# Lab-LVM/imagenet-models

Hardware: AMD Instinct MI355X
Metric: images/sec (whole node) GA-ConvNeXt-T 3x224x224 bf16 training step (higher is better)
Workload: dtype bf16; 1 GPU; ga_convnext_tiny_768 train step (fwd + GA loss lam=-0.8 + bwd + all-reduce + adamw lr=0), batch 256/GPU, drop_path 0.2, synthetic 3x224x224; global_batch=256, parallelism=dp1, dist_backend=none, grad_exchange=torch, allreduce_buckets=0

## Files before the change

imagenet-models_amd/_lib.py:

```python
import ctypes as C
import os

_HERE = os.path.dirname(os.path.abspath(__file__))
LIB_PATH = os.environ.get('GAEXT_LIB') or os.path.join(_HERE, 'csrc', 'libgaext.so')

GA_F32, GA_BF16 = 0, 1
ACT_NONE, ACT_GELU, ACT_RELU = 0, 1, 2
A_PLAIN, A_PATCH2, A_STEM4_NCHW, A_CONV3, A_CONV3S2, A_NEIGH2 = 0, 1, 2, 3, 4, 5
C_PLAIN, C_UNPATCH2 = 0, 1

vp, i32, i64, f32 = C.c_void_p, C.c_int, C.c_int64, C.c_float


class GemmDesc(C.Structure):
    _fields_ = [
        ('M', i32), ('N', i32), ('K', i32), ('batch', i32), ('dtype', i32),
        ('A', vp), ('lda', i64), ('strideA', i64), ('a_batch_mod', i32), ('a_kind', i32),
        ('a_H', i32), ('a_W', i32), ('a_C', i32), ('a_act', i32),
        ('B', vp), ('ldb', i64), ('strideB', i64),
        ('C', vp), ('ldc', i64), ('strideC', i64), ('c_kind', i32),
        ('c_H', i32), ('c_W', i32), ('c_C', i32), ('c_f32', i32), ('C2', vp), ('c2_mode', i32),
        ('alpha', f32), ('bias', vp), ('strideBias', i64), ('act', i32),
        ('H', vp), ('ldh', i64), ('strideH', i64), ('h_is_deriv', i32),
        ('rowscale', vp), ('rows_per_scale', i32),
        ('R', vp), ('ldr', i64), ('strideR', i64), ('relu_after', i32),
        ('colsum', vp), ('colsumsq', vp), ('strideCol', i64),
    ]


class WgradDesc(C.Structure):
    _fields_ = [
        ('M', i32), ('N', i32), ('K', i32), ('batch', i32), ('dtype', i32),
        ('Y', vp), ('ldy', i64), ('strideY', i64),
        ('X', vp), ('ldx', i64), ('strideX', i64), ('x_batch_mod', i32), ('x_kind', i32),
        ('x_H', i32), ('x_W', i32), ('x_C', i32), ('x_act', i32),
        ('dW', vp), ('ldw', i64), ('strideW', i64),
        ('dbias', vp), ('strideDbias', i64),
        ('alpha', f32), ('split_m', i32), ('accumulate', i32), ('workspace', vp), ('ws_bytes', i64),
    ]


class WprepDesc(C.Structure):
    _fields_ = [
        ('w', vp), ('G', i32), ('Co', i32), ('Ci', i32), ('KH', i32), ('KW', i32),
        ('rs', vp), ('cs', vp), ('row_perm', vp), ('dtype', i32),
        ('out', vp), ('ldo', i64), ('outT', vp), ('ldt', i64), ('flip', i32), ('stem', i32), ('t_cols', i32),
    ]


class WunfoldDesc(C.Structure):
    _fields_ = [
        ('G', vp), ('ldg', i64), ('gb', vp), ('W', vp), ('b', vp), ('rs', vp), ('cs', vp), ('v', vp), ('row_perm', vp),
        ('N', i32), ('Ci', i32), ('KH', i32), ('KW', i32), ('stem', i32),
        ('dW', vp), ('db', vp), ('d_rs', vp), ('d_cs', vp), ('d_v', vp),
    ]


class SmallDesc(C.Structure):
    _fields_ = [('kind', i32), ('y', vp), ('x', vp), ('a', f32), ('n', i64), ('R', i32), ('C', i32), ('accumulate', i32),
                ('b', vp), ('rs', vp), ('v', vp), ('row_perm', vp)]


class CswinAttnDesc(C.Structure):
    _fields_ = [('B', i32), ('reso', i32), ('C', i32), ('heads', i32), ('nbranch', i32),
                ('Hs', i32 * 2), ('Ws', i32 * 2), ('lepe_w', vp * 2), ('lepe_b', vp * 2),
                ('scale', f32), ('dtype', i32), ('qkv', vp), ('ldq', i64), ('out', vp), ('ldo', i64)]


class MlpDesc(C.Structure):
    _fields_ = [('X', vp), ('ldx', i64), ('W1', vp), ('ldw1', i64), ('b1', vp), ('W2', vp), ('ldw2', i64), ('b2', vp),
                ('R', vp), ('ldr', i64), ('rowscale', vp), ('rows_per_scale', i32), ('Y', vp), ('ldy', i64),
                ('M', i64), ('C', i32), ('H', i32), ('dtype', i32)]


class MlpBwdDesc(C.Structure):
    _fields_ = [('X', vp), ('ldx', i64), ('DY', vp), ('lddy', i64), ('W1', vp), ('ldw1', i64), ('b1', vp),
                ('W2T', vp), ('ldw2t', i64), ('W1T', vp), ('ldw1t', i64), ('A', vp), ('lda', i64), ('DH', vp), ('lddh', i64),
                ('DX', vp), ('lddx', i64), ('M', i64), ('C', i32), ('H', i32), ('dtype', i32),
                ('dW1', vp), ('ldw', i64), ('db1', vp), ('partials', vp), ('partials_bytes', C.c_size_t), ('max_blocks', i32)]


class SmallLinearDesc(C.Structure):
    _fields_ = [('rows', i32), ('groups', i32), ('Ng', i32), ('Kg', i32), ('A', vp), ('lda', i64), ('a_gstride', i64), ('a_perm', vp),
                ('W', vp), ('bias', vp), ('col_scale', vp), ('rowscale', vp), ('rows_per_scale', i32), ('R', vp), ('ldr', i64),
                ('Y', vp), ('ldy', i64), ('Yraw', vp), ('dtype', i32)]


class AttnDesc(C.Structure):
    _fields_ = [('B', i32), ('N', i32), ('H', i32), ('hd', i32), ('scale', f32), ('dtype', i32), ('qkv', vp), ('ldq', i64),
                ('out', vp), ('ldo', i64), ('lse', vp)]


_SIGS = {
    'ga_version': ([], i32),
    'ga_last_error': ([C.c_char_p, C.c_size_t], i32),
    'ga_device_info': ([C.POINTER(i32), C.POINTER(i32), C.POINTER(i32)], i32),
    'ga_comm_unique_id': ([vp], i32),
    'ga_comm_init': ([C.POINTER(vp), i32, i32, vp], i32),
    'ga_comm_destroy': ([vp], i32),
    'ga_comm_info': ([vp, C.POINTER(i32), C.POINTER(i32)], i32),
    'ga_allreduce_workspace': ([i64, i32], C.c_size_t),
    'ga_allreduce_bucket': ([vp, vp, i64, i32, f32, vp, C.c_size_t, vp], i32),
    'ga_reduce_scatter_bucket': ([vp, vp, vp, i64, f32, vp], i32),
    'ga_allgather_bucket': ([vp, vp, vp, i64, vp], i32),
    'ga_comm_broadcast': ([vp, vp, i64, i32, vp], i32),
    'ga_set_knob': ([C.c_char_p, i32], i32),
    'ga_unset_knob': ([C.c_char_p], i32),
    'ga_config_string': ([C.c_char_p, C.c_size_t], i32),
    'ga_gemm': ([C.POINTER(GemmDesc), vp], i32),
    'ga_wgrad': ([C.POINTER(WgradDesc), vp], i32),
    'ga_weight_prep': ([C.POINTER(WprepDesc), vp], i32),
    'ga_bias_fold': ([vp, vp, vp, vp, vp, vp, i32, i32, vp], i32),
    'ga_weight_unfold': ([C.POINTER(WunfoldDesc), vp], i32),
    'ga_dwconv7_fwd': ([vp, vp, vp, vp, i32, i32, i32, i32, i32, vp], i32),
    'ga_dwconv7_bwd_data': ([vp, vp, vp, vp, i32, i32, i32, i32, i32, vp], i32),
    'ga_dwconv7_bwd_data2': ([vp, vp, vp, vp, vp, vp, i32, i32, i32, i32, i32, vp], i32),
    'ga_dwconv7_bwd_weight': ([vp, vp, vp, vp, i32, i32, i32, i32, i32, vp, C.c_size_t, vp], i32),
    'ga_dwconv7_bwd_weight_workspace': ([i32, i32, i32, i32, i32], C.c_size_t),
    'ga_dwconv3_fwd': ([vp, vp, vp, i32, i32, i32, i32, i32, vp, vp, i32, vp], i32),
    'ga_dwconv3_bwd_data': ([vp, vp, vp, i32, i32, i32, i32, i32, i32, vp], i32),
    'ga_dwconv3_bwd_weight': ([vp, vp, vp, i32, i32, i32, i32, i32, i32, vp, C.c_size_t, vp], i32),
    'ga_dwconv3_bwd_weight_workspace': ([i32, i32, i32, i32, i32, i32], C.c_size_t),
    'ga_maxpool3s2_fwd': ([vp, vp, vp, i32, i32, i32, i32, i32, vp], i32),
    'ga_maxpool3s2_bwd': ([vp, vp, vp, i32, i32, i32, i32, i32, i32, vp], i32),
    'ga_bn_gelu_fwd': ([vp, vp, vp, vp, i64, i32, i32, vp], i32),
    'ga_bn_gelu_bwd_workspace': ([i64, i32], C.c_size_t),
    'ga_bn_gelu_bwd_reduce': ([vp, vp, vp, vp, vp, vp, vp, vp, i64, i32, i32, vp, C.c_size_t, vp], i32),
    'ga_bn_gelu_bwd_apply': ([vp, vp, vp, vp, vp, vp, vp, vp, vp, i64, vp, i64, i32, i32, vp], i32),
    'ga_se_bn_fwd': ([vp, i32, vp, vp, vp, vp, vp, vp, vp, vp, vp, vp, vp, vp, vp, vp, i32, i32, i32, i32, vp], i32),
    'ga_se_bn_bwd': ([vp, vp, vp, vp, vp, vp, vp, vp, i32, vp, vp, vp, vp, vp, vp, vp, vp, vp, vp, vp, vp, vp, vp, vp, vp, vp, vp, vp,
                      vp, vp, i32, i32, i32, vp], i32),
    'ga_se_residual_fwd': ([vp, vp, vp, vp, vp, vp, vp, vp, vp, i32, i32, i32, i32, vp], i32),
    'ga_se_residual_bwd_a': ([vp, vp, vp, vp, vp, vp, vp, vp, i32, i32, i32, i32, vp], i32),
    'ga_se_residual_bwd_b': ([vp, vp, vp, vp, vp, vp, vp, vp, vp, vp, vp, i32, i32, i32, i32, vp], i32),
    'ga_subsample2_fwd': ([vp, vp, i32, i32, i32, i32, i32, vp], i32),
    'ga_subsample2_bwd': ([vp, vp, i32, i32, i32, i32, i32, i32, vp], i32),
    'ga_wgrad_workspace': ([C.POINTER(WgradDesc)], C.c_size_t),
    'ga_layernorm_fwd': ([vp, vp, vp, vp, vp, vp, i64, i32, f32, i32, vp], i32),
    'ga_layernorm_bwd': ([vp, vp, vp, vp, vp, vp, vp, vp, vp, i64, i32, i32, i32, vp], i32),
    'ga_layernorm_bwd_dp': ([vp, vp, vp, vp, vp, vp, vp, vp, vp, i64, i32, i32, vp, vp, i64, i32, vp], i32),
    'ga_bn_finalize': ([vp, vp, i64, vp, vp, f32, f32, vp, vp, vp, vp, vp, vp, i32, i32, vp], i32),
    'ga_affine_act': ([vp, vp, vp, vp, vp, i64, vp, i64, i32, i32, i32, i64, vp], i32),
    'ga_bn_bwd_reduce': ([vp, vp, vp, vp, vp, vp, i64, vp, vp, i64, i32, i32, i64, vp], i32),
    'ga_bn_bwd_apply': ([vp, vp, vp, vp, vp, vp, vp, vp, vp, i64, i64, vp, i64, i32, i32, i64, i64, vp], i32),
    'ga_pool_concat_fwd': ([vp, vp, i32, i32, i32, i32, i32, i32, i32, i32, i32, i32, vp], i32),
    'ga_pool_concat_bwd': ([vp, vp, vp, i32, i32, i32, i32, i32, i32, i32, i32, i32, i32, vp], i32),
    'ga_spatial_sum': ([vp, vp, vp, i32, i32, i32, f32, i32, vp], i32),
    'ga_se_mlp_fwd': ([vp, vp, vp, vp, vp, vp, vp, i32, i32, i32, vp], i32),
    'ga_se_mlp_bwd': ([vp, vp, vp, vp, vp, vp, vp, f32, vp, vp, vp, vp, i32, i32, i32, vp], i32),
    'ga_chan_scale': ([vp, vp, vp, vp, i32, i32, i32, i32, vp], i32),
    'ga_gram_pack_fwd': ([vp, vp, vp, i32, i32, i32, i32, i32, vp], i32),
    'ga_gram_pack_bwd': ([vp, vp, vp, vp, i32, i32, i32, i32, i32, vp], i32),
    'ga_gram_f64_fwd_workspace': ([i32, i32], C.c_size_t),
    'ga_gram_f64_bwd_workspace': ([i32, i32], C.c_size_t),
    'ga_gram_f64_fwd': ([vp, vp, vp, vp, C.c_size_t, i32, i32, i32, i32, i32, i32, i32, vp], i32),
    'ga_gram_f64_bwd': ([vp, vp, vp, vp, vp, vp, C.c_size_t, i32, i32, i32, i32, i32, i32, i32, vp], i32),
    'ga_token_cat': ([vp, vp, vp, i32, i32, i32, i32, vp], i32),
    'ga_token_split': ([vp, vp, vp, i32, i32, i32, i32, i32, i32, vp], i32),
    'ga_class_attn_fwd': ([vp, vp, vp, vp, i32, i32, i32, i32, f32, i32, vp], i32),
    'ga_class_attn_bwd': ([vp, vp, vp, vp, vp, vp, i32, i32, i32, i32, f32, i32, vp], i32),
    'ga_class_attn_fwd2': ([vp, vp, vp, i64, vp, vp, i32, i32, i32, i32, f32, i32, vp], i32),
    'ga_class_attn_bwd2': ([vp, vp, vp, vp, i64, vp, vp, vp, vp, i32, i32, i32, i32, f32, i32, vp], i32),
    'ga_loss_fwd_bwd': ([vp, vp, vp, vp, i32, i32, i32, f32, i32, f32, f32, i32, vp], i32),
    'ga_heads_topk': ([vp, i32, i32, i32, i32, vp, vp, vp], i32),
    'ga_sgd_step': ([vp, vp, vp, vp, i64, i32, f32, vp], i32),
    'ga_adamw_step': ([vp, vp, vp, vp, vp, i64, f32, vp], i32),
    'ga_weight_prep_batch': ([vp, i32, vp], i32),
    'ga_weight_unfold_batch': ([vp, i32, vp], i32),
    'ga_small_batch': ([vp, i32, vp], i32),
    'ga_cswin_attn_fwd': ([C.POINTER(CswinAttnDesc), vp], i32),
    'ga_cswin_attn_bwd_workspace': ([C.POINTER(CswinAttnDesc)], C.c_size_t),
    'ga_cswin_attn_bwd': ([C.POINTER(CswinAttnDesc), vp, vp, vp, C.c_size_t, vp], i32),
    'ga_cswin_lepe_wgrad_reduce': ([C.POINTER(CswinAttnDesc), vp, vp, vp, vp, vp, vp], i32),
    'ga_cswin_lepe_wgrad': ([C.POINTER(CswinAttnDesc), vp, vp, vp, vp, vp, vp], i32),
    'ga_layernorm_gelu_fwd': ([vp, vp, vp, vp, vp, vp, i64, i32, f32, i32, vp], i32),
    'ga_layernorm_gelu_bwd': ([vp, vp, vp, vp, vp, vp, vp, vp, vp, i64, i32, i32, vp], i32),
    'ga_nchw3_to_nhwc8': ([vp, vp, i32, i32, i32, i32, vp], i32),
    'ga_convw_pack': ([vp, vp, i32, i32, i32, i32, i64, i32, vp], i32),
    'ga_convw_unpack_grad': ([vp, vp, i32, i32, i32, i32, i64, vp], i32),
    'ga_conv3s2_dgrad_prep': ([vp, vp, i32, i32, i64, i32, vp], i32),
    'ga_gram_pack_fwd2': ([vp, vp, vp, i32, i32, i32, i32, i32, i32, vp], i32),
    'ga_gram_pack_bwd2': ([vp, vp, vp, vp, i32, i32, i32, i32, i32, i32, vp], i32),
    'ga_map_tokens_fwd': ([vp, vp, i32, i32, i32, i32, i32, vp], i32),
    'ga_map_tokens_bwd': ([vp, vp, i32, i32, i32, i32, i32, vp], i32),
    'ga_class_attn_mt_fwd': ([vp, vp, vp, i64, vp, vp, vp, i32, i32, i32, i32, i32, f32, i32, vp], i32),
    'ga_class_attn_mt_bwd': ([vp, vp, vp, vp, i64, vp, vp, vp, vp, vp, i64, i32, i32, i32, i32, i32, f32, i32, vp], i32),
    'ga_class_attn_mt_ia_fwd': ([vp, vp, vp, i64, vp, vp, vp, vp, vp, vp, vp, i32, i32, i32, i32, i32, f32, i32, vp], i32),
    'ga_class_attn_mt_ia_bwd': ([vp, vp, vp, vp, i64, vp, vp, vp, vp, vp, vp, vp, vp, i64, vp, vp, vp, vp, i32, i32, i32, i32, i32, f32, i32,
                                 vp], i32),
    'ga_map_loss_fwd_bwd': ([vp, vp, vp, vp, vp, vp, i32, i32, i32, f32, i32, f32, f32, i32, vp], i32),
    'ga_gelu_fwd': ([vp, vp, i64, i32, vp], i32),
    'ga_gelu_bwd': ([vp, vp, vp, i64, i32, vp], i32),
    'ga_relu_drop': ([vp, vp, vp, vp, i64, i32, vp], i32),
    'ga_mask_mul': ([vp, vp, vp, vp, i64, i32, vp], i32),
    'ga_copy2d': ([vp, i64, vp, i64, i64, i32, i32, i32, vp], i32),
    'ga_dropout_mask_sample': ([vp, i64, f32, C.c_uint64, vp, vp], i32),
    'ga_drop_path_sample': ([vp, vp, i32, i32, C.c_uint64, vp, vp], i32),
    'ga_loss_dense_fwd_bwd': ([vp, vp, vp, vp, vp, vp, vp, i32, i32, i32, f32, i32, f32, f32, f32, i32, vp], i32),
    'ga_u8_normalize': ([vp, vp, i32, i32, i32, i32, C.POINTER(f32), C.POINTER(f32), vp], i32),
    'ga_input_erase': ([vp, i32, vp, i32, i32, i32, i32, C.POINTER(f32), C.POINTER(f32), vp, i32, i32, C.c_uint64, C.c_uint64, vp], i32),
    'ga_mixup_batch': ([vp, vp, i32, i32, i32, i32, C.c_double, i32, i32, i32, i32, i32, vp], i32),
    'ga_mixup_target': ([vp, vp, i32, i32, C.c_double, C.c_double, vp], i32),
    'ga_agc_clip': ([vp, vp, vp, i32, f32, f32, vp], i32),
    'ga_small_linear_fwd': ([C.POINTER(SmallLinearDesc), vp], i32),
    'ga_small_linear_bwd': ([C.POINTER(SmallLinearDesc), vp, vp, i32, vp, vp, vp, vp], i32),
    'ga_colstats': ([vp, i64, i32, i32, vp, vp, i32, vp], i32),
    'ga_pad_copy_f32': ([vp, vp, i64, i64, i64, i64, i32, vp], i32),
    'ga_pad_copy': ([vp, vp, i64, i64, i64, i64, i32, i32, vp], i32),
    'ga_stem4_ln_fwd': ([vp, vp, i64, vp, vp, vp, vp, vp, vp, vp, i32, i32, i32, i32, f32, vp], i32),
    'ga_blockdiag_f32': ([vp, vp, i64, i32, i32, i32, i64, i32, i32, vp], i32),
    'ga_pad_groups_f32': ([vp, vp, i64, i64, i32, i32, i32, i32, i32, i32, vp], i32),
    'ga_attn_fwd': ([C.POINTER(AttnDesc), vp], i32),
    'ga_attn_bwd_workspace': ([C.POINTER(AttnDesc)], C.c_size_t),
    'ga_attn_bwd': ([C.POINTER(AttnDesc), vp, vp, vp, C.c_size_t, vp], i32),
    'ga_patchify': ([vp, vp, i32, i32, i32, i32, i32, i32, vp], i32),
    'ga_vit_embed_fwd': ([vp, vp, vp, vp, i32, i32, i32, i32, vp], i32),
    'ga_vit_embed_bwd': ([vp, vp, vp, vp, i32, i32, i32, i32, vp], i32),
    'ga_patchify_strided': ([vp, vp, i32, i32, i32, i32, i32, i32, i32, vp], i32),
    'ga_pos_add_fwd': ([vp, vp, vp, i32, i32, i32, i32, vp], i32),
    'ga_pos_add_bwd': ([vp, vp, i32, i32, i32, i32, vp], i32),
    'ga_dwpool_fwd': ([vp, vp, vp, vp, i32, i32, i32, i32, i32, i32, vp], i32),
    'ga_dwpool_bwd_data': ([vp, vp, vp, i32, i32, i32, i32, i32, i32, vp], i32),
    'ga_dwpool_bwd_weight': ([vp, vp, vp, vp, i32, i32, i32, i32, i32, i32, vp], i32),
    'ga_resize_concat_fwd': ([vp, vp, i32, i32, i32, i32, i32, i32, i64, i32, i32, vp], i32),
    'ga_resize_concat_bwd': ([vp, vp, i32, i32, i32, i32, i32, i32, i64, i32, i32, vp], i32),
    'ga_rows_bcast': ([vp, vp, i32, i32, i32, f32, i32, vp], i32),
    'ga_token_gap_fwd': ([vp, vp, i32, i32, i32, i32, vp], i32),
    'ga_token_gap_bwd': ([vp, vp, i32, i32, i32, i32, vp], i32),
    'ga_mlp_supported': ([i32, i32, i32], i32),
    'ga_mlp_fwd': ([C.POINTER(MlpDesc), vp], i32),
    'ga_mlp_bwd': ([C.POINTER(MlpBwdDesc), vp], i32),
    'ga_mlp_bwd_wgrad_supported': ([i32, i32, i32], i32),
    'ga_mlp_bwd_partials': ([C.POINTER(MlpBwdDesc)], C.c_size_t),
    'ga_memset': ([vp, i32, C.c_size_t, vp], i32),
    'ga_transpose_f32': ([vp, vp, i32, i32, i32, vp], i32),
    'ga_axpy_f32': ([vp, vp, f32, i64, vp], i32),
    'ga_lerp_f32': ([vp, vp, f32, i64, vp], i32),
    'ga_sumsq_f32': ([vp, i64, vp, vp], i32),
    'ga_lamb_stage1': ([vp, vp, vp, vp, vp, vp, vp, vp, i32, vp, vp], i32),
    'ga_lamb_stage2': ([vp, vp, vp, vp, i32, vp, vp], i32),
    'ga_clip_grad_f32': ([vp, i64, vp, f32, i32, vp], i32),
    'ga_rowscale': ([vp, vp, vp, i64, i64, i32, vp], i32),
    'ga_cast_from_f32': ([vp, vp, i64, i32, vp], i32),
    'ga_cast_to_f32': ([vp, vp, i64, i32, vp], i32),
}

_lib = None


def load():
    global _lib
    if _lib is not None:
        return _lib
    if not os.path.exists(LIB_PATH):
        raise RuntimeError(f'libgaext.so not found at {LIB_PATH}: build it with `make -C {os.path.dirname(LIB_PATH)}` '
                           f'(there is no CPU fallback for the product path)')
    lib = C.CDLL(LIB_PATH)
    for name, (argtypes, restype) in _SIGS.items():
        fn = getattr(lib, name)
        fn.argtypes = argtypes
        fn.restype = restype
    _lib = lib
    return lib


def last_error():
    buf = C.create_string_buffer(512)
    load().ga_last_error(buf, 512)
    return buf.value.decode(errors='replace')


def config_string():
    buf = C.create_string_buffer(1024)
    load().ga_config_string(buf, 1024)
    s = buf.value.decode(errors='replace')
    host = sorted(k for k in os.environ if k.startswith(('GAEXT_', 'GA_FUSED_MLP')) and k != 'GAEXT_LIB')
    known = {'GAEXT_ASYNC_WGRAD', 'GAEXT_FWD_SPLIT', 'GAEXT_PAR_BRANCH', 'GAEXT_FWD_SKEW', 'GAEXT_FUSE_DP', 'GAEXT_HEAD_STREAMS',
             'GA_FUSED_MLP', 'GAEXT_SMALL_SINGLE', 'GAEXT_SYNC_DEBUG', 'GAEXT_MLP_WG1'}
    for k in host:
        if k in known:
            s += f' host:{k}={os.environ[k]}'
    if os.environ.get('GAEXT_LIB'):
        s += f' lib={os.environ["GAEXT_LIB"]}'
    return s


class knobs:

    def __init__(self, **kv):
        self.kv = kv

    def __enter__(self):
        lib = load()
        for k, v in self.kv.items():
            check(lib.ga_set_knob(k.encode(), int(v)), f'ga_set_knob({k})')
        return self

    def __exit__(self, *exc):
        lib = load()
        for k in self.kv:
            lib.ga_unset_knob(k.encode())
        return False


def check(rc, what):
    if rc != 0:
        raise RuntimeError(f'libgaext {what} failed (code {rc}): {last_error()}')


def exported_symbols():
    return sorted(_SIGS)
```

imagenet-models_amd/csrc/mlp.hip:

```cpp
#include <stdlib.h>
#include <algorithm>
#include "common.h"

namespace {

constexpr int BM = 128;

__device__ __forceinline__ void lds_barrier() { asm volatile("s_waitcnt lgkmcnt(0)\n\ts_barrier" ::: "memory"); }

__device__ __forceinline__ unsigned slab_off(int r, int c) { return r * 64 + ((c ^ ((r >> 2) & 3)) << 4); }

__device__ __forceinline__ bf16x8_t frag(const unsigned char* slab, int r0, int lane) {
    return *reinterpret_cast<const bf16x8_t*>(slab + slab_off(r0 + (lane & 15), lane >> 4));
}

template <int ROWS, int KS, int NTHR>
__device__ __forceinline__ void stage_rows(unsigned char* dst, const bf16_t* src, long ld, long row0, long limit, int tid) {
    constexpr int CPR = KS * 4, NP = ROWS * CPR / NTHR;
    static_assert(ROWS * CPR % NTHR == 0, "tile must split evenly over the threads");
    u32x4_t v[NP];
#pragma unroll
    for (int i = 0; i < NP; ++i) {
        const int idx = tid + NTHR * i;
        const int r = idx / CPR, c = idx - r * CPR;
        v[i] = u32x4_t{0, 0, 0, 0};
        if (row0 + r < limit) v[i] = __builtin_nontemporal_load(reinterpret_cast<const u32x4_t*>(src + (row0 + r) * ld + c * 8));
    }
#pragma unroll
    for (int i = 0; i < NP; ++i) {
        const int idx = tid + NTHR * i;
        const int r = idx / CPR, c = idx - r * CPR;
        *reinterpret_cast<u32x4_t*>(dst + (c >> 2) * ROWS * 64 + slab_off(r, c & 3)) = v[i];
    }
}

template <int C, int NTHR> struct RowPre {
    static constexpr int P8 = C / 8, RG = NTHR / P8, NR = (64 + RG - 1) / RG;
};
template <int C, int NTHR> using PreArr = u32x4_t[BM / 64][RowPre<C, NTHR>::NR];
template <int C, int NTHR>
__device__ __forceinline__ void rows_prefetch(PreArr<C, NTHR>& v, const bf16_t* R, long ldr, long m0, long M) {
    using P = RowPre<C, NTHR>;
    const int c8 = threadIdx.x % P::P8, rg = threadIdx.x / P::P8;
#pragma unroll
    for (int piece = 0; piece < BM / 64; ++piece)
#pragma unroll
        for (int it = 0; it < P::NR; ++it) {
            const int row = rg + it * P::RG;
            const long m = m0 + piece * 64 + row;
            v[piece][it] = u32x4_t{0, 0, 0, 0};
            if (rg < P::RG && row < 64 && m < M) v[piece][it] = __builtin_nontemporal_load(reinterpret_cast<const u32x4_t*>(R + m * ldr + c8 * 8));
        }
}

template <int C, int NTHR, int NWM, int TM>
__device__ __forceinline__ void store_rows(float* Cs, const f32x4_t (&acc)[C / 32][TM], int wm, int wn, int lane, long m0, long M,
                                           const float* bias, const float* rowscale, int rps, bool has_r,
                                           const PreArr<C, NTHR>& pre, bf16_t* Y, long ldy, int tid) {
    constexpr int LDC = C + 4, P8 = C / 8, RG = NTHR / P8, WROWS = 16 * TM, WPH = 64 / WROWS;
    constexpr int NR = (64 + RG - 1) / RG;
    const int c8 = tid % P8, rg = tid / P8;
    float bv[8];
#pragma unroll
    for (int j = 0; j < 8; ++j) bv[j] = bias ? bias[c8 * 8 + j] : 0.f;
#pragma unroll
    for (int piece = 0; piece < NWM / WPH; ++piece) {
        if (piece) __syncthreads();
        if (wm / WPH == piece) {
#pragma unroll
            for (int tn = 0; tn < C / 32; ++tn)
#pragma unroll
                for (int tm = 0; tm < TM; ++tm) {
                    const int row = (wm % WPH) * WROWS + 16 * tm + (lane & 15), col = wn * (C / 2) + 16 * tn + 4 * (lane >> 4);
                    *reinterpret_cast<f32x4_t*>(Cs + row * LDC + col) = acc[tn][tm];
                }
        }
        __syncthreads();
        if (rg < RG) {
#pragma unroll
            for (int it = 0; it < NR; ++it) {
                const int row = rg + it * RG;
                const long m = m0 + piece * 64 + row;
                if (row >= 64 || m >= M) break;
                const f32x4_t a = *reinterpret_cast<const f32x4_t*>(Cs + row * LDC + c8 * 8);
                const f32x4_t b = *reinterpret_cast<const f32x4_t*>(Cs + row * LDC + c8 * 8 + 4);
                float v[8] = {a[0], a[1], a[2], a[3], b[0], b[1], b[2], b[3]};
#pragma unroll
                for (int j = 0; j < 8; ++j) v[j] += bv[j];
                if (rowscale) {
                    const float s = rowscale[m / rps];
#pragma unroll
                    for (int j = 0; j < 8; ++j) v[j] *= s;
                }
                if (has_r) {
                    float r[8];
                    const u32x4_t q = pre[piece][it];
                    unpack8(make_uint4(q.x, q.y, q.z, q.w), r);
#pragma unroll
                    for (int j = 0; j < 8; ++j) v[j] += r[j];
                }
                store8_nt(Y + m * ldy + c8 * 8, v);
            }
        }
    }
}

template <int C, int HC>
__global__ __launch_bounds__(256, 2) void mlp_fwd_kernel(const ga_mlp_desc d) {
    constexpr int KS1 = C / 32, KS2 = HC / 32, TN1 = HC / 32, TN2 = C / 32;
    constexpr int XS = KS1 * BM * 64, W1S = KS1 * HC * 64, AS = KS2 * BM * 64;
    constexpr int NI = HC * C / 8 / 256;
    static_assert(HC * C / 8 % 256 == 0, "weight chunk must split evenly");
    extern __shared__ __attribute__((aligned(16))) unsigned char smem[];
    unsigned char* Xs = smem;
    unsigned char* W1s = Xs + XS;
    unsigned char* As = W1s + W1S;
    unsigned char* W2s = As + AS;
    float* B1s = reinterpret_cast<float*>(W2s + KS2 * C * 64);
    const int tid = threadIdx.x, lane = tid & 63, wave = tid >> 6, wm = wave >> 1, wn = wave & 1, g = lane >> 4;
    const long m0 = (long)blockIdx.x * BM;
    const bf16_t* W1 = reinterpret_cast<const bf16_t*>(d.W1);
    const bf16_t* W2 = reinterpret_cast<const bf16_t*>(d.W2);

    u32x4_t w1r[NI], w2r[NI];
    auto w_load = [&](int j0) {
#pragma unroll
        for (int i = 0; i < NI; ++i) {
            const int idx = tid + 256 * i;
            const int r1 = idx / (KS1 * 4), c1 = idx - r1 * (KS1 * 4);
            w1r[i] = *reinterpret_cast<const u32x4_t*>(W1 + (long)(j0 + r1) * d.ldw1 + c1 * 8);
            const int r2 = idx / (HC / 8), c2 = idx - r2 * (HC / 8);
            w2r[i] = *reinterpret_cast<const u32x4_t*>(W2 + (long)r2 * d.ldw2 + j0 + c2 * 8);
        }
    };
    auto w1_store = [&]() {
#pragma unroll
        for (int i = 0; i < NI; ++i) {
            const int idx = tid + 256 * i;
            const int r1 = idx / (KS1 * 4), c1 = idx - r1 * (KS1 * 4);
            *reinterpret_cast<u32x4_t*>(W1s + (c1 >> 2) * HC * 64 + slab_off(r1, c1 & 3)) = w1r[i];
        }
    };
    auto w2_store = [&]() {
#pragma unroll
        for (int i = 0; i < NI; ++i) {
            const int idx = tid + 256 * i;
            const int r2 = idx / (HC / 8), c2 = idx - r2 * (HC / 8);
            *reinterpret_cast<u32x4_t*>(W2s + (c2 >> 2) * C * 64 + slab_off(r2, c2 & 3)) = w2r[i];
        }
    };

    w_load(0);
    stage_rows<BM, KS1, 256>(Xs, reinterpret_cast<const bf16_t*>(d.X), d.ldx, m0, d.M, tid);
    for (int i = tid; i < 4 * C; i += 256) B1s[i] = d.b1[i];
    w1_store();
    w2_store();
    __syncthreads();

    f32x4_t y[TN2][4];
#pragma unroll
    for (int i = 0; i < TN2; ++i)
#pragma unroll
        for (int j = 0; j < 4; ++j) y[i][j] = f32x4_t{0.f, 0.f, 0.f, 0.f};
    auto round = [&](const int j0, const bool more) __attribute__((always_inline)) {
        if (more) w_load(j0 + HC);
        f32x4_t h[TN1][4];
#pragma unroll
        for (int i = 0; i < TN1; ++i)
#pragma unroll
            for (int j = 0; j < 4; ++j) h[i][j] = f32x4_t{0.f, 0.f, 0.f, 0.f};
#pragma unroll
        for (int ks = 0; ks < KS1; ++ks) {
            bf16x8_t xf[4];
#pragma unroll
            for (int tm = 0; tm < 4; ++tm) xf[tm] = frag(Xs + ks * BM * 64, wm * 64 + 16 * tm, lane);
#pragma unroll
            for (int tn = 0; tn < TN1; ++tn) {
                const bf16x8_t wf = frag(W1s + ks * HC * 64, wn * (HC / 2) + 16 * tn, lane);
#pragma unroll
                for (int tm = 0; tm < 4; ++tm) h[tn][tm] = __builtin_amdgcn_mfma_f32_16x16x32_bf16(wf, xf[tm], h[tn][tm], 0, 0, 0);
            }
        }
#pragma unroll
        for (int tn = 0; tn < TN1; ++tn) {
            const int nl = wn * (HC / 2) + 16 * tn + 4 * g;
            const float4 b = *reinterpret_cast<const float4*>(B1s + j0 + nl);
            const float bb[4] = {b.x, b.y, b.z, b.w};
#pragma unroll
            for (int tm = 0; tm < 4; ++tm) {
                float a[4], unused;
#pragma unroll
                for (int r = 0; r < 4; ++r) gelu_both_fast(h[tn][tm][r] + bb[r], a[r], unused);
                const int row = wm * 64 + 16 * tm + (lane & 15);
                uint2 p;
                p.x = pack2bf(a[0], a[1]);
                p.y = pack2bf(a[2], a[3]);
                *reinterpret_cast<uint2*>(As + (nl >> 5) * BM * 64 + slab_off(row, (nl & 31) >> 3) + (nl & 7) * 2) = p;
            }
        }
        lds_barrier();
#pragma unroll
        for (int ks = 0; ks < KS2; ++ks) {
            bf16x8_t af[4];
#pragma unroll
            for (int tm = 0; tm < 4; ++tm) af[tm] = frag(As + ks * BM * 64, wm * 64 + 16 * tm, lane);
#pragma unroll
            for (int tn = 0; tn < TN2; ++tn) {
                const bf16x8_t wf = frag(W2s + ks * C * 64, wn * (C / 2) + 16 * tn, lane);
#pragma unroll
                for (int tm = 0; tm < 4; ++tm) y[tn][tm] = __builtin_amdgcn_mfma_f32_16x16x32_bf16(wf, af[tm], y[tn][tm], 0, 0, 0);
            }
        }
        if (more) w1_store();
        lds_barrier();
        if (more) w2_store();
    };
    for (int j0 = 0; j0 + HC < d.H; j0 += HC) round(j0, true);
    u32x4_t rpre[BM / 64][RowPre<C, 256>::NR];
    if (d.R) rows_prefetch<C, 256>(rpre, reinterpret_cast<const bf16_t*>(d.R), d.ldr, m0, d.M);
    round(d.H - HC, false);
    store_rows<C, 256, 2, 4>(reinterpret_cast<float*>(smem), y, wm, wn, lane, m0, d.M, d.b2, d.rowscale, d.rows_per_scale,
                             d.R != nullptr, rpre, reinterpret_cast<bf16_t*>(d.Y), d.ldy, tid);
}

template <int C, int HC> constexpr int fwd_lds() {
    constexpr int ab = (C / 32) * BM * 64 + (C / 32) * HC * 64 + (HC / 32) * BM * 64 + (HC / 32) * C * 64 + 16 * C;
    constexpr int st = 64 * (C + 4) * 4;
    return ab > st ? ab : st;
}

__device__ __forceinline__ unsigned tr_off(int lane, int hf, int u0) {
    const int i = lane & 15, row = 8 * (lane >> 4) + 4 * hf + (i >> 2);
    return slab_off(row, u0 + ((i & 3) >> 1)) + 8 * (i & 1);
}
__device__ __forceinline__ bf16x8_t tr_frag(const unsigned char* lo, const unsigned char* hi) {
    s16x4_t v[2];
    v[0] = __builtin_amdgcn_ds_read_tr16_b64_v4i16((__attribute__((address_space(3))) s16x4_t*)lo);
    v[1] = __builtin_amdgcn_ds_read_tr16_b64_v4i16((__attribute__((address_space(3))) s16x4_t*)hi);
    return *reinterpret_cast<const bf16x8_t*>(&v[0]);
}

template <int C, int HC, bool WG>
__global__ __launch_bounds__(512, 1) void mlp_bwd_kernel(const ga_mlp_bwd_desc d) {
    constexpr int KS1 = C / 32, KS2 = HC / 32, TN1 = HC / 32, TN2 = C / 32;
    constexpr int XS = KS1 * BM * 64, WS = KS1 * HC * 64, TS = KS2 * BM * 64;
    constexpr int NPC = HC * C / 8, NI = (NPC + 511) / 512;
    constexpr int NCH = 4 * C / HC;
    static_assert(!WG || (HC == 64 && C == 96), "the in-kernel weight gradient is laid out for 4 x 6 tiles over 8 waves");
    extern __shared__ __attribute__((aligned(16))) unsigned char smem[];
    unsigned char* Xs = smem;
    unsigned char* Ds = Xs + XS;
    unsigned char* W1s = Ds + XS;
    unsigned char* W2Ts = W1s + WS;
    unsigned char* W1Ts = W2Ts + WS;
    unsigned char* DHs = W1Ts + KS2 * C * 64;
    unsigned char* A2s = DHs + TS;
    float* B1s = reinterpret_cast<float*>(A2s + TS);
    const int tid = threadIdx.x, lane = tid & 63, wave = tid >> 6, wm = wave >> 1, wn = wave & 1, g = lane >> 4;
    const bf16_t* W1 = reinterpret_cast<const bf16_t*>(d.W1);
    const bf16_t* W2T = reinterpret_cast<const bf16_t*>(d.W2T);
    const bf16_t* W1T = reinterpret_cast<const bf16_t*>(d.W1T);
    bf16_t* Aout = reinterpret_cast<bf16_t*>(d.A);
    bf16_t* DHout = reinterpret_cast<bf16_t*>(d.DH);

    u32x4_t w1r[NI], w2r[NI], w3r[NI];
    auto w_load = [&](int j0) {
#pragma unroll
        for (int i = 0; i < NI; ++i) {
            const int idx = NPC % 512 == 0 ? tid + 512 * i : min(tid + 512 * i, NPC - 1);
            const int r1 = idx / (KS1 * 4), c1 = idx - r1 * (KS1 * 4);
            w1r[i] = *reinterpret_cast<const u32x4_t*>(W1 + (long)(j0 + r1) * d.ldw1 + c1 * 8);
            w2r[i] = *reinterpret_cast<const u32x4_t*>(W2T + (long)(j0 + r1) * d.ldw2t + c1 * 8);
            const int r3 = idx / (HC / 8), c3 = idx - r3 * (HC / 8);
            w3r[i] = *reinterpret_cast<const u32x4_t*>(W1T + (long)r3 * d.ldw1t + j0 + c3 * 8);
        }
    };
    auto w12_store = [&]() {
#pragma unroll
        for (int i = 0; i < NI; ++i) {
            const int idx = NPC % 512 == 0 ? tid + 512 * i : min(tid + 512 * i, NPC - 1);
            const int r1 = idx / (KS1 * 4), c1 = idx - r1 * (KS1 * 4);
            const unsigned o = (c1 >> 2) * HC * 64 + slab_off(r1, c1 & 3);
            *reinterpret_cast<u32x4_t*>(W1s + o) = w1r[i];
            *reinterpret_cast<u32x4_t*>(W2Ts + o) = w2r[i];
        }
    };
    auto w3_store = [&]() {
#pragma unroll
        for (int i = 0; i < NI; ++i) {
            const int idx = NPC % 512 == 0 ? tid + 512 * i : min(tid + 512 * i, NPC - 1);
            const int r3 = idx / (HC / 8), c3 = idx - r3 * (HC / 8);
            *reinterpret_cast<u32x4_t*>(W1Ts + (c3 >> 2) * C * 64 + slab_off(r3, c3 & 3)) = w3r[i];
        }
    };

    constexpr int NDW = WG ? NCH : 1;
    f32x4_t dw[NDW][3];
    float bsum[NDW];
    unsigned tra[2];
    if constexpr (WG) {
#pragma unroll
        for (int i = 0; i < NDW; ++i) {
            bsum[i] = 0.f;
#pragma unroll
            for (int j = 0; j < 3; ++j) dw[i][j] = f32x4_t{0.f, 0.f, 0.f, 0.f};
        }
        tra[0] = tr_off(lane, 0, 0);
        tra[1] = tr_off(lane, 1, 0);
    }
    const int wu = __builtin_amdgcn_readfirstlane(wave);
    auto tr_blk = [&](const unsigned char* img, int blk, int ks) __attribute__((always_inline)) {
        const unsigned o = (unsigned)(img - smem) + (blk >> 1) * BM * 64 + ks * 2048, x = (blk & 1) << 5;
        return tr_frag(smem + ((tra[0] ^ x) + o), smem + ((tra[1] ^ x) + o));
    };

    for (int i = tid; i < 4 * C; i += 512) B1s[i] = d.b1[i];
    const long ntiles = (d.M + BM - 1) / BM;
    long tile = blockIdx.x;
    w_load(0);
    while (true) {
        const long m0 = tile * BM;
        const bool first = !WG || tile == (long)blockIdx.x;
        const bool next_tile = WG && tile + (long)gridDim.x < ntiles;
        int ttid = tid;
        if constexpr (WG) asm volatile("" : "+v"(ttid));
        stage_rows<BM, KS1, 512>(Xs, reinterpret_cast<const bf16_t*>(d.X), d.ldx, m0, d.M, ttid);
        stage_rows<BM, KS1, 512>(Ds, reinterpret_cast<const bf16_t*>(d.DY), d.lddy, m0, d.M, ttid);
        if (first) {
            w12_store();
            w3_store();
        }
        __syncthreads();

        f32x4_t dx[TN2][2];
#pragma unroll
        for (int i = 0; i < TN2; ++i)
#pragma unroll
            for (int j = 0; j < 2; ++j) dx[i][j] = f32x4_t{0.f, 0.f, 0.f, 0.f};

        auto wg_chunk = [&](f32x4_t (&dwc)[3], float& bs) __attribute__((always_inline)) {
            typedef __attribute__((ext_vector_type(2))) __bf16 bf16x2_t;
            const bf16x2_t ones2 = {(__bf16)1.0f, (__bf16)1.0f};
#pragma unroll
            for (int ks = 0; ks < BM / 32; ++ks) {
                const bf16x8_t hf8 = tr_blk(DHs, wu >> 1, ks);
#pragma unroll
                for (int tc = 0; tc < 3; ++tc) {
                    const bf16x8_t xf8 = tr_blk(Xs, 3 * (wu & 1) + tc, ks);
                    dwc[tc] = __builtin_amdgcn_mfma_f32_16x16x32_bf16(hf8, xf8, dwc[tc], 0, 0, 0);
                }
                if ((wu & 1) == 0) {
#pragma unroll
                    for (int j = 0; j < 4; ++j)
                        bs = __builtin_amdgcn_fdot2_f32_bf16(bf16x2_t{hf8[2 * j], hf8[2 * j + 1]}, ones2, bs, false);
                }
            }
        };
        auto chunk = [&](const int j0, const bool more, const int jn) __attribute__((always_inline)) {
            if (more) w_load(jn);
            f32x4_t h[TN1][2], t[TN1][2];
#pragma unroll
            for (int i = 0; i < TN1; ++i)
#pragma unroll
                for (int j = 0; j < 2; ++j) h[i][j] = t[i][j] = f32x4_t{0.f, 0.f, 0.f, 0.f};
#pragma unroll
            for (int ks = 0; ks < KS1; ++ks) {
                bf16x8_t xf[2], df[2];
#pragma unroll
                for (int tm = 0; tm < 2; ++tm) {
                    xf[tm] = frag(Xs + ks * BM * 64, wm * 32 + 16 * tm, lane);
                    df[tm] = frag(Ds + ks * BM * 64, wm * 32 + 16 * tm, lane);
                }
#pragma unroll
                for (int tn = 0; tn < TN1; ++tn) {
                    const bf16x8_t w1f = frag(W1s + ks * HC * 64, wn * (HC / 2) + 16 * tn, lane);
                    const bf16x8_t w2f = frag(W2Ts + ks * HC * 64, wn * (HC / 2) + 16 * tn, lane);
#pragma unroll
                    for (int tm = 0; tm < 2; ++tm) {
                        h[tn][tm] = __builtin_amdgcn_mfma_f32_16x16x32_bf16(w1f, xf[tm], h[tn][tm], 0, 0, 0);
                        t[tn][tm] = __builtin_amdgcn_mfma_f32_16x16x32_bf16(w2f, df[tm], t[tn][tm], 0, 0, 0);
                    }
                }
            }
#pragma unroll
            for (int tn = 0; tn < TN1; ++tn) {
                const int nl = wn * (HC / 2) + 16 * tn + 4 * g;
                const float4 b = *reinterpret_cast<const float4*>(B1s + j0 + nl);
                const float bb[4] = {b.x, b.y, b.z, b.w};
#pragma unroll
                for (int tm = 0; tm < 2; ++tm) {
                    float a[4], dh[4];
#pragma unroll
                    for (int r = 0; r < 4; ++r) {
                        float gr;
                        gelu_both_fast(h[tn][tm][r] + bb[r], a[r], gr);
                        dh[r] = t[tn][tm][r] * gr;
                    }
                    const int row = wm * 32 + 16 * tm + (lane & 15);
                    const unsigned o = (nl >> 5) * BM * 64 + slab_off(row, (nl & 31) >> 3) + (nl & 7) * 2;
                    uint2 p;
                    p.x = pack2bf(a[0], a[1]);
                    p.y = pack2bf(a[2], a[3]);
                    *reinterpret_cast<uint2*>(A2s + o) = p;
                    p.x = pack2bf(dh[0], dh[1]);
                    p.y = pack2bf(dh[2], dh[3]);
                    *reinterpret_cast<uint2*>(DHs + o) = p;
                }
            }
            lds_barrier();
#pragma unroll
            for (int ks = 0; ks < KS2; ++ks) {
                bf16x8_t af[2];
#pragma unroll
                for (int tm = 0; tm < 2; ++tm) af[tm] = frag(DHs + ks * BM * 64, wm * 32 + 16 * tm, lane);
#pragma unroll
                for (int tn = 0; tn < TN2; ++tn) {
                    const bf16x8_t wf = frag(W1Ts + ks * C * 64, wn * (C / 2) + 16 * tn, lane);
#pragma unroll
                    for (int tm = 0; tm < 2; ++tm) dx[tn][tm] = __builtin_amdgcn_mfma_f32_16x16x32_bf16(wf, af[tm], dx[tn][tm], 0, 0, 0);
                }
            }
            if constexpr (WG) {
                static_assert(NDW == 1 || NDW == 6, "one case per chunk");
                switch (j0 / HC) {
                    case 0: wg_chunk(dw[0], bsum[0]); break;
                    case 1: wg_chunk(dw[1 % NDW], bsum[1 % NDW]); break;
                    case 2: wg_chunk(dw[2 % NDW], bsum[2 % NDW]); break;
                    case 3: wg_chunk(dw[3 % NDW], bsum[3 % NDW]); break;
                    case 4: wg_chunk(dw[4 % NDW], bsum[4 % NDW]); break;
                    default: wg_chunk(dw[5 % NDW], bsum[5 % NDW]); break;
                }
            }
            if (Aout || DHout) {
                constexpr int PPR = HC / 8, NP = BM * PPR / 512;
                static_assert(BM * PPR % 512 == 0, "chunk rows must split evenly");
                int ctid = tid;
                if constexpr (WG) asm volatile("" : "+v"(ctid));
#pragma unroll
                for (int i = 0; i < NP; ++i) {
                    const int idx = ctid + 512 * i;
                    const int r = idx / PPR, c = idx - r * PPR;
                    const long m = m0 + r;
                    if (m < d.M) {
                        const unsigned o = (c >> 2) * BM * 64 + slab_off(r, c & 3);
                        if (Aout) store16_nt(Aout + m * d.lda + j0 + c * 8, *reinterpret_cast<const uint4*>(A2s + o));
                        if (DHout) store16_nt(DHout + m * d.lddh + j0 + c * 8, *reinterpret_cast<const uint4*>(DHs + o));
                    }
                }
            }
            if (more) w12_store();
            lds_barrier();
            if (more) w3_store();
        };
        for (int j0 = 0; j0 < d.H; j0 += HC) {
            const bool last = j0 + HC >= d.H;
            chunk(j0, !last || next_tile, last ? 0 : j0 + HC);
        }
        u32x4_t nopre[BM / 64][RowPre<C, 512>::NR];
#pragma unroll
        for (int i = 0; i < BM / 64; ++i)
#pragma unroll
            for (int j = 0; j < RowPre<C, 512>::NR; ++j) nopre[i][j] = u32x4_t{0, 0, 0, 0};
        int stid = tid;
        if constexpr (WG) asm volatile("" : "+v"(stid));
        store_rows<C, 512, 4, 2>(reinterpret_cast<float*>(smem), dx, stid >> 7, (stid >> 6) & 1, stid & 63, m0, d.M, nullptr, nullptr, 1,
                                 false, nopre, reinterpret_cast<bf16_t*>(d.DX), d.lddx, stid);
        if (!next_tile) break;
        tile += gridDim.x;
        __syncthreads();
    }
    if constexpr (WG) {
        float* P = d.partials + (long)blockIdx.x * (4 * C * C + 4 * C);
        int etid = tid;
        asm volatile("" : "+v"(etid));
        const int lane = etid & 63, g = lane >> 4, jt = wu >> 1;
#pragma unroll
        for (int ch = 0; ch < NCH; ++ch) {
#pragma unroll
            for (int tc = 0; tc < 3; ++tc)
#pragma unroll
                for (int r = 0; r < 4; ++r)
                    P[(ch * HC + 16 * jt + 4 * g + r) * C + 16 * (3 * (wu & 1) + tc) + (lane & 15)] = dw[ch][tc][r];
            float v = bsum[ch];
            v += __shfl_xor(v, 16, 64);
            v += __shfl_xor(v, 32, 64);
            if ((wu & 1) == 0 && lane < 16) P[4 * C * C + ch * HC + 16 * jt + lane] = v;
        }
    }
}

__global__ __launch_bounds__(256) void mlp_bwd_wg_reduce_kernel(const float* __restrict__ part, int nparts, int n, int nw, int C,
                                                                float* __restrict__ dW1, long ldw, float* __restrict__ db1) {
    __shared__ float4 sh[3][64];
    const int q = threadIdx.x >> 6;
    const long i = ((long)blockIdx.x * 64 + (threadIdx.x & 63)) * 4;
    float4 a = make_float4(0.f, 0.f, 0.f, 0.f);
    if (i < n) {
#pragma unroll 4
        for (int s = q; s < nparts; s += 4) {
            const float4 b = *reinterpret_cast<const float4*>(part + (long)s * n + i);
            a.x += b.x; a.y += b.y; a.z += b.z; a.w += b.w;
        }
    }
    if (q) sh[q - 1][threadIdx.x & 63] = a;
    __syncthreads();
    if (q || i >= n) return;
#pragma unroll
    for (int s = 0; s < 3; ++s) {
        const float4 b = sh[s][threadIdx.x];
        a.x += b.x; a.y += b.y; a.z += b.z; a.w += b.w;
    }
    float* dst = i < nw ? dW1 + (i / C) * ldw + (i % C) : db1 + (i - nw);
    dst[0] += a.x; dst[1] += a.y; dst[2] += a.z; dst[3] += a.w;
}

template <int C, int HC> constexpr int bwd_lds() {
    return 2 * (C / 32) * BM * 64 + 2 * (C / 32) * HC * 64 + (HC / 32) * C * 64 + 2 * (HC / 32) * BM * 64 + 16 * C;
}

bool aligned16(const void* p) { return (reinterpret_cast<uintptr_t>(p) & 15) == 0; }

template <typename K> bool set_lds(K kern, size_t bytes) {
    return bytes <= 65536 ||
           hipFuncSetAttribute(reinterpret_cast<const void*>(kern), hipFuncAttributeMaxDynamicSharedMemorySize, (int)bytes) == hipSuccess;
}

}

extern "C" int ga_mlp_supported(int C, int H, int dtype) { return dtype == GA_BF16 && H == 4 * C && (C == 96 || C == 192); }

extern "C" int ga_mlp_fwd(const ga_mlp_desc* d, ga_stream_t stream) {
    GA_REQUIRE(d && d->X && d->W1 && d->b1 && d->W2 && d->Y && d->M > 0, "ga_mlp_fwd: null / empty descriptor");
    GA_REQUIRE(ga_mlp_supported(d->C, d->H, d->dtype), "ga_mlp_fwd: C=%d H=%d dtype=%d has no fused form (ga_mlp_supported)", d->C,
               d->H, d->dtype);
    GA_REQUIRE(aligned16(d->X) && aligned16(d->W1) && aligned16(d->W2) && aligned16(d->Y) && aligned16(d->b1) &&
                   (!d->R || aligned16(d->R)) && d->ldx % 8 == 0 && d->ldw1 % 8 == 0 && d->ldw2 % 8 == 0 && d->ldy % 8 == 0 &&
                   (!d->R || d->ldr % 8 == 0) && d->ldx >= d->C && d->ldw1 >= d->C && d->ldw2 >= d->H && d->ldy >= d->C,
               "ga_mlp_fwd: operands must be 16-byte aligned with leading dimensions in multiples of 8");
    GA_REQUIRE(!d->rowscale || d->rows_per_scale > 0, "ga_mlp_fwd: rows_per_scale");
    hipStream_t s = reinterpret_cast<hipStream_t>(stream);
    const unsigned grid = (unsigned)((d->M + BM - 1) / BM);
    if (d->C == 96) {
        constexpr int lds = fwd_lds<96, 64>();
        GA_REQUIRE(set_lds(mlp_fwd_kernel<96, 64>, lds), "ga_mlp_fwd: LDS");
        hipLaunchKernelGGL((mlp_fwd_kernel<96, 64>), dim3(grid), dim3(256), lds, s, *d);
    } else {
        constexpr int lds = fwd_lds<192, 32>();
        GA_REQUIRE(set_lds(mlp_fwd_kernel<192, 32>, lds), "ga_mlp_fwd: LDS");
        hipLaunchKernelGGL((mlp_fwd_kernel<192, 32>), dim3(grid), dim3(256), lds, s, *d);
    }
    return ga_check_launch("ga_mlp_fwd");
}

extern "C" int ga_mlp_bwd_wgrad_supported(int C, int H, int dtype) { return dtype == GA_BF16 && C == 96 && H == 4 * C; }

namespace {

int num_cus() {
    static int n = [] {
        int c = 256;
        ga_device_info(&c, nullptr, nullptr);
        return c;
    }();
    return n;
}

int wg_grid(const ga_mlp_bwd_desc* d) {
    constexpr int lds = bwd_lds<96, 64>();
    static const int resident = [] {
        auto kern = mlp_bwd_kernel<96, 64, true>;
        if (!set_lds(kern, lds)) return 0;
        int n = 0;
        if (hipOccupancyMaxActiveBlocksPerMultiprocessor(&n, kern, 512, lds) != hipSuccess || n < 1) n = 1;
        return n * num_cus();
    }();
    long grid = resident;
    if (d->max_blocks > 0) grid = std::min<long>(grid, d->max_blocks);
    return (int)std::min<long>(grid, (d->M + BM - 1) / BM);
}

}

extern "C" size_t ga_mlp_bwd_partials(const ga_mlp_bwd_desc* d) {
    if (!d || d->M <= 0 || !ga_mlp_bwd_wgrad_supported(d->C, d->H, d->dtype)) return 0;
    return (size_t)wg_grid(d) * ((size_t)d->H * d->C + d->H) * sizeof(float);
}

extern "C" int ga_mlp_bwd(const ga_mlp_bwd_desc* d, ga_stream_t stream) {
    GA_REQUIRE(d && d->X && d->DY && d->W1 && d->b1 && d->W2T && d->W1T && d->DX && d->M > 0, "ga_mlp_bwd: null / empty descriptor");
    GA_REQUIRE(ga_mlp_supported(d->C, d->H, d->dtype), "ga_mlp_bwd: C=%d H=%d dtype=%d has no fused form (ga_mlp_supported)", d->C,
               d->H, d->dtype);
    GA_REQUIRE(aligned16(d->X) && aligned16(d->DY) && aligned16(d->W1) && aligned16(d->W2T) && aligned16(d->W1T) &&
                   aligned16(d->A) && aligned16(d->DH) && aligned16(d->DX) && aligned16(d->b1) && d->ldx % 8 == 0 &&
                   d->lddy % 8 == 0 && d->ldw1 % 8 == 0 && d->ldw2t % 8 == 0 && d->ldw1t % 8 == 0 && (!d->A || d->lda % 8 == 0) &&
                   (!d->DH || d->lddh % 8 == 0) && d->lddx % 8 == 0 && d->ldx >= d->C && d->lddy >= d->C && d->ldw1 >= d->C &&
                   d->ldw2t >= d->C && d->ldw1t >= d->H && (!d->A || d->lda >= d->H) && (!d->DH || d->lddh >= d->H) &&
                   d->lddx >= d->C,
               "ga_mlp_bwd: operands must be 16-byte aligned with leading dimensions in multiples of 8");
    hipStream_t s = reinterpret_cast<hipStream_t>(stream);
    if (d->dW1) {
        GA_REQUIRE(ga_mlp_bwd_wgrad_supported(d->C, d->H, d->dtype),
                   "ga_mlp_bwd: dW1 is accumulated in the kernel at C=96 only, not C=%d H=%d dtype=%d (ga_mlp_bwd_wgrad_supported)",
                   d->C, d->H, d->dtype);
        GA_REQUIRE(d->db1 && d->partials && aligned16(d->partials) && d->ldw >= d->C && d->max_blocks >= 0,
                   "ga_mlp_bwd: dW1 needs db1, 16-byte aligned partials and ldw >= C");
        constexpr int lds = bwd_lds<96, 64>();
        const int grid = wg_grid(d);
        GA_REQUIRE(grid > 0, "ga_mlp_bwd: LDS");
        const int n = d->H * d->C + d->H;
        GA_REQUIRE(d->partials_bytes >= (size_t)grid * n * sizeof(float), "ga_mlp_bwd: partials holds %zu bytes, %zu needed (ga_mlp_bwd_partials)",
                   (size_t)d->partials_bytes, (size_t)grid * n * sizeof(float));
        hipLaunchKernelGGL((mlp_bwd_kernel<96, 64, true>), dim3(grid), dim3(512), lds, s, *d);
        hipLaunchKernelGGL(mlp_bwd_wg_reduce_kernel, dim3((n / 4 + 63) / 64), dim3(256), 0, s, d->partials, grid, n, d->H * d->C, d->C,
                           d->dW1, (long)d->ldw, d->db1);
        return ga_check_launch("ga_mlp_bwd");
    }
    const unsigned grid = (unsigned)((d->M + BM - 1) / BM);
    if (d->C == 96) {
        constexpr int lds = bwd_lds<96, 64>();
        GA_REQUIRE(set_lds(mlp_bwd_kernel<96, 64, false>, lds), "ga_mlp_bwd: LDS");
        hipLaunchKernelGGL((mlp_bwd_kernel<96, 64, false>), dim3(grid), dim3(512), lds, s, *d);
    } else {
        constexpr int lds = bwd_lds<192, 32>();
        GA_REQUIRE(set_lds(mlp_bwd_kernel<192, 32, false>, lds), "ga_mlp_bwd: LDS");
        hipLaunchKernelGGL((mlp_bwd_kernel<192, 32, false>), dim3(grid), dim3(512), lds, s, *d);
    }
    return ga_check_launch("ga_mlp_bwd");
}
```

imagenet-models_amd/engine.py:

```python
import contextlib
import os

import torch

from . import ops
from .ops import (A_CONV3, A_PATCH2, A_STEM4_NCHW, ACT_GELU, ASYNC_LANE, C_UNPATCH2, GA_BF16, GA_F32, Plan)


def pad8(n):
    return (n + 7) // 8 * 8


def tap_indices(nblocks, naggre):
    taps = []
    if nblocks > 5:
        for i in range(nblocks):
            if (i + 1) % (nblocks // (naggre + 1)) == 0 and len(taps) < naggre:
                taps.append(i)
    return taps


class GAFunction(torch.autograd.Function):

    @staticmethod
    def forward(ctx, eng, x, anchor):
        ctx.eng = eng
        return eng.forward(x)

    @staticmethod
    def backward(ctx, dlogits):
        ctx.eng.backward(dlogits)
        return None, None, None


class GAEngine:
    def __init__(self, model, batch, training, mode):
        self.m = model
        self.cfg = model.cfg
        self.B = batch
        self.training = training
        self.dt = GA_BF16 if mode == 'bf16' else GA_F32
        self.tdt = ops.torch_dtype(self.dt)
        flat = model.flat_state()
        self.dev = flat['params'].device
        self.P = dict(model.named_parameters())
        self.Bf = dict(model.named_buffers())
        self.bufs = {}
        self.tmps = {}
        self.async_wgrad = os.environ.get('GAEXT_ASYNC_WGRAD', '1') != '0'
        self.mlp_wg1 = os.environ.get('GAEXT_MLP_WG1', '1') != '0'
        self.fwd_split = max(1, int(os.environ.get('GAEXT_FWD_SPLIT', '2')))
        self.par_branch = os.environ.get('GAEXT_PAR_BRANCH', '1') != '0'
        self.fwd_skew = int(os.environ.get('GAEXT_FWD_SKEW', '-1'))
        self._chain = None
        self._cur_stage = 0
        self._bwd_seq = 0
        self._pre_dyz = {}
        self.fuse_dp = os.environ.get('GAEXT_FUSE_DP', '1') != '0'
        self.sync_bn = getattr(model, 'sync_bn_comm', None)
        self.W = {}
        self.weights_dirty = True
        self.anchor = torch.zeros((), device=self.dev, requires_grad=True)
        self.input_descs = []
        self.blocks = {}
        self.x_ref = None
        self.img = 224
        self.dp_rates = self._drop_path_rates()
        self.dp_scale = {}
        if training:
            sites = [pre for pre, r in self.dp_rates.items() if r > 0]
            if sites:
                self.dp_all = torch.ones(len(sites), batch, device=self.dev)
                self.dp_keep = torch.tensor([1.0 - self.dp_rates[p] for p in sites], device=self.dev)
                self.dp_counter = torch.zeros(1, dtype=torch.int64, device=self.dev)
                self.dp_plan = Plan(name='droppath')
                self.dp_plan.drop_path_sample(self.dp_all, self.dp_keep, len(sites), batch, torch.initial_seed(), self.dp_counter)
                for i, pre in enumerate(sites):
                    self.dp_scale[pre] = self.dp_all[i]
        self.arena = None
        self.arena_off = 0
        if training:
            self.arena = torch.zeros(int(flat['total'] * 1.15) + (1 << 20) + self._arena_extra(), device=self.dev)
        self._nbt = [t for n, t in self.Bf.items() if n.endswith('num_batches_tracked')]
        self.prep = Plan(name='prep', defer_small=True)
        self.fwd = Plan(name='fwd')
        self.bwd = Plan(name='bwd', defer_small=True) if training else None
        self.bn_pool = torch.zeros(1 << 16, device=self.dev)
        self.bn_pool_off = 0
        self.bott_prefix = 'stages.4.'
        self.ppad, self.pgrad = {}, {}
        self.pad_gmlp = os.environ.get('GAEXT_PAD_GMLP', '1') != '0'
        self._build()
        assert not self.pgrad or getattr(self, '_unpadded', False), 'padded parameter gradients were never copied back'

    def buf(self, name, shape, dtype=None, zero=False):
        dtype = dtype or self.tdt
        if name not in self.bufs:
            self.bufs[name] = (torch.zeros if zero else torch.empty)(shape, dtype=dtype, device=self.dev)
        t = self.bufs[name]
        assert tuple(t.shape) == tuple(shape) and t.dtype == dtype, name
        return t

    def _chains(self):
        n = self.fwd_split if self.B >= 2 * self.fwd_split else 1
        if n <= 1:
            return [(0, 0, self.B)]
        per = self.B // n
        cuts = [s_ * per for s_ in range(n)] + [self.B]
        return [(1 + s_, cuts[s_], cuts[s_ + 1]) for s_ in range(n)]

    def _fsplits(self, HW):
        ch = getattr(self, '_chain', None)
        if ch is None:
            return [(0, 0, self.B * HW, 0, self.B)]
        lane, b0, b1 = ch
        return [(lane, b0 * HW, b1 * HW, b0, b1)]

    @contextlib.contextmanager
    def _wlane(self):
        Bk = self.bwd
        prev = Bk.lane
        if self.async_wgrad and prev == 0:
            Bk.lane = ASYNC_LANE
        try:
            yield
        finally:
            Bk.lane = prev

    def tmp(self, tag, shape, dtype=None):
        dtype = dtype or self.tdt
        key = (getattr(self, 'tmp_prefix', '') + tag, tuple(shape), dtype)
        if key not in self.tmps:
            self.tmps[key] = torch.empty(shape, dtype=dtype, device=self.dev)
        return self.tmps[key]

    def act(self, name, shape, dtype=None):
        return self.buf(name, shape, dtype)

    def blk_act(self, name, shape, dtype=None):
        return self.buf(name, shape, dtype) if self.training else self.tmp(name.rsplit('.', 1)[-1], shape, dtype)

    def gbuf(self, shape):
        n = 1
        for s in shape:
            n *= s
        off = (self.arena_off + 63) // 64 * 64
        assert off + n <= self.arena.numel(), 'gradient scratch arena too small'
        self.arena_off = off + n
        return self.arena[off:off + n].view(shape)

    def grad(self, name):
        return self.P[name].grad

    def _drop_path_rates(self):
        dep = self.cfg['depths']
        rate = self.cfg['drop_path_rate']
        pts = torch.linspace(0, rate, sum(dep)).split(list(dep))
        out = {}
        for i in range(4):
            for j in range(dep[i]):
                out[f'stages.{i}.blocks.{j}.'] = float(pts[i][j])
        out['stages.4.'] = float(rate)
        for k in range(self.cfg['branches']):
            out[f'gram_layer.{k}.blocks.0.'] = float(pts[-1][0])
            out[f'ga.{k}.'] = 0.0
        return out

    def sample_drop_path(self):
        if self.dp_scale:
            self.dp_plan.run()

    def set_drop_path_masks(self, masks):
        for pre, t in self.dp_scale.items():
            t.copy_(masks[pre].to(self.dev).float())

    NAMES = dict(stem_conv='stem.0.', stem_ln='stem.1.', ds_ln='stages.{i}.downsample.0.', ds_conv='stages.{i}.downsample.1.',
                 block='stages.{i}.blocks.{j}.', dw='conv_dw.', fc1='mlp.fc1.', fc2='mlp.fc2.')

    def _build(self):
        cfg = self.cfg
        d = cfg['dims']
        B, T, F = self.B, self.training, self.fwd
        dt = self.dt
        feats, taps, stage_in, _ = self._build_trunk()
        Hc = 14
        M4 = B * Hc * Hc
        ctot = sum(d[:-1]) + d[2] * cfg['naggre']
        cat = self.act('agg.cat', (M4, ctot))
        segs = [(feats[0][0], feats[0][1], d[0], 0), (feats[1][0], feats[1][1], d[1], 0)]
        segs += [(t, feats[2][1], d[2], 0) for t in taps]
        segs += [(feats[2][0], feats[2][1], d[2], 0), (feats[3][0], feats[3][1], d[3], 1)]
        off = 0
        self.agg_segs = []
        for src, hw, c, mode in segs:
            F.pool_concat_fwd(src, cat, B, hw, hw, c, Hc, Hc, ctot, off, mode, dt, label=f'agg.{off}')
            self.agg_segs.append((src, hw, c, mode, off))
            off += c
        assert off == ctot
        x4 = self._bottleneck_fwd(cat, M4, ctot, d[4])
        self.cout = d[4]
        self._build_heads(x4, M4, Hc)
        if T:
            self._build_backward(feats, taps, stage_in, x4, M4, ctot)
# ... 106 lines not shown
            tk = self.tok
            tk['E2'], tk['ld'] = E2, K * E2
            tk['W'] = self.buf('w.ga.kv_all', (K * E2, cout))
            tk['WT'] = self.buf('wT.ga.kv_all', (cout, K * E2)) if T else None
            tk['b'] = self.buf('w.ga.bkv_all', (K * E2,), torch.float32)
            P = self.P
            for k in range(K):
                pre = f'ga.{k}.'
                pk, pv = P[pre + 'attn.k.weight'], P[pre + 'attn.v.weight']
                assert pv.data_ptr() == pk.data_ptr() + pk.numel() * 4, 'k/v weights must be adjacent in the flat buffer'
                pk = self._pw(pre + 'attn.k.weight')
                self.prep.weight_prep(pk, 1, E2, cout, 1, 1, dt, out=tk['W'][k * E2:], ldo=cout,
                                      outT=tk['WT'][:, k * E2:] if T else None, ldt=K * E2 if T else 0,
                                      cs=P[pre + 'norm1.weight'], t_cols=E2, label='prep.' + pre + 'kv')
                self.prep.bias_fold(pk, None, None, P[pre + 'norm1.bias'], tk['b'][k * E2:], E2, cout)
            tk['kv'] = self.act('ga.kv_all', (M4, K * E2))
            F.gemm(tk['xn'], tk['W'], tk['kv'], M4, K * E2, cout, dt, bias=tk['b'], label='ga.kv_all')
        self._contract_all_fwd(x4, M4)
        fa = self.fc_all = dict(x=self.act('fc.all.x', (K, B, cout)))
        ldn = pad8(NC)
        fa['W'] = self.buf('w.fc.all', (K, NC, cout))
        fa['WT'] = self.buf('wT.fc.all', (K, cout, ldn)) if T else None
        fa['b'] = self.buf('w.fc.ball', (K, NC), torch.float32)
        for k in range(K):
            self.prep.weight_prep(self.P[f'fc.{k}.weight'], 1, NC, cout, 1, 1, dt, out=fa['W'][k], ldo=cout,
                                  outT=fa['WT'][k] if T else None, ldt=ldn if T else 0, label=f'prep.fc.{k}')
            self.prep.bias_fold(None, self.P[f'fc.{k}.bias'], None, None, fa['b'][k], NC, cout)
        self.head_lanes = int(os.environ.get('GAEXT_HEAD_STREAMS', '5')) if self.shared_tok else 1
        for k in range(K):
            if self.head_lanes > 1:
                F.lane, self.tmp_prefix = 1 + k % self.head_lanes, f'h{k}.'
            self.heads.append(self._head_fwd(k, x4, M4, cout, Hc))
        F.lane, self.tmp_prefix = 0, ''
        F.gemm(fa['x'], fa['W'], self.logits, B, NC, cout, dt, batch=K, strideA=B * cout, strideB=NC * cout, strideC=B * NC,
               bias=fa['b'], strideBias=NC, c_f32=True, label='fc.all')

    def _arena_extra(self):
        cfg = self.cfg
        d = cfg.get('dims')
        if not d or len(d) < 5 or any(k not in cfg for k in ('gram_dim', 'gram_groups', 'mlp_groups', 'dim_embed', 'num_heads', 'branches')):
            return 0
        cout, g, groups = d[4], cfg['gram_dim'], cfg['gram_groups']
        if cout % (8 * groups) == 0 and cout % (8 * cfg['mlp_groups']) == 0 and (cfg['dim_embed'] // max(cfg['num_heads'], 1)) % 8 == 0:
            return 0
        cp = cout + 8 * max(groups, cfg['mlp_groups'])
        return cfg['branches'] * (cp * (g * (g + 1) // 2 // groups + 8) + 8 * cp * cp // cfg['mlp_groups'] + 4 * cp * 512) + (1 << 20)

    def _pw(self, name):
        return self.ppad[name][0] if name in self.ppad else self.P[name]

    def _pg(self, name):
        if name not in self.ppad:
            return self.grad(name)
        if name not in self.pgrad:
            self.pgrad[name] = self.gbuf(tuple(self.ppad[name][0].shape))
        return self.pgrad[name]

    def _pad_groups(self, name, R, Cdim, RG, RGp, CG, CGp):
        if name not in self.ppad:
            buf = self.buf('pad.' + name, (R // RG * RGp, Cdim // CG * CGp), torch.float32, zero=True)
            self.prep.pad_groups_f32(self.P[name], buf, R, Cdim, RG, RGp, CG, CGp, label='prep.pad.' + name)
            self.ppad[name] = (buf, 'groups', (R, Cdim, RG, RGp, CG, CGp))
        return self.ppad[name][0]

    def _unpad_all(self):
        self._unpadded = True
        for name, g in self.pgrad.items():
            _, kind, a = self.ppad[name]
            if kind == 'copy':
                rows, cols, lds, ldd = a
                self.bwd.pad_copy_f32(g, self.grad(name), rows, cols, ldd, lds, accumulate=True, label=name + '.unpad')
            else:
                self.bwd.pad_groups_f32(g, self.grad(name), *a, unpad=True, accumulate=True, label=name + '.unpad')

    def _contract_all_fwd(self, x4, M4):
        cfg, T, F, dt, cout = self.cfg, self.training, self.fwd, self.dt, self.cout
        K = cfg['branches']
        g_ = cfg['gram_dim']
        gc = self.gcon = dict(ld=K * g_)
        gc['W'] = self.buf('w.gram_contraction.all', (K * g_, cout))
        gc['WT'] = self.buf('wT.gram_contraction.all', (cout, K * g_)) if T else None
        gc['b'] = self.buf('w.gram_contraction.ball', (K * g_,), torch.float32)
        gc['s'], gc['q'] = self._bn_pool(K * g_), self._bn_pool(K * g_)
        for k in range(K):
            pre = f'gram_contraction.{k}.'
            self.prep.weight_prep(self.P[pre + '0.weight'], 1, g_, cout, 1, 1, dt, out=gc['W'][k * g_:], ldo=cout,
                                  outT=gc['WT'][:, k * g_:] if T else None, ldt=K * g_ if T else 0, t_cols=g_,
                                  label='prep.' + pre + 'w')
            self.prep.bias_fold(None, self.P[pre + '0.bias'], None, None, gc['b'][k * g_:], g_, cout)
        gc['out'] = self.act('gram_contraction.all.out', (M4, K * g_))
        F.gemm(x4, gc['W'], gc['out'], M4, K * g_, cout, dt, bias=gc['b'], colsum=gc['s'] if T else None,
               colsumsq=gc['q'] if T else None, label='gram_contraction.all')

    @staticmethod
    def _last_desc(plan):
        for obj in reversed(plan.keep):
            if hasattr(obj, '_fields_'):
                return obj
        raise RuntimeError('no descriptor')

    def _w_plain(self, name, Co, Ci, KH, KW, stem=False, need_T=True, flip=False, groups=1, rs=None, cs=None,
                 row_perm=None, ldo=None, key=None, src=None):
        key = key or name
        if key in self.W:
            return self.W[key]
        KK = Ci * KH * KW
        ldo = ldo or pad8(KK)
        out = self.buf('w.' + key, (groups * Co, ldo))
        outT = None
        ldt = 0
        if need_T and self.training:
            if flip:
                ldt = pad8(KH * KW * Co)
                outT = self.buf('wT.' + key, (groups * Ci, ldt))
            else:
                ldt = pad8(Co)
                outT = self.buf('wT.' + key, (groups * KK, ldt))
            self.W[key + '.T'] = outT
        self.prep.weight_prep(self.P[name] if src is None else src, groups, Co, Ci, KH, KW, self.dt, out=out, ldo=ldo, outT=outT, ldt=ldt, rs=rs,
                              cs=cs, flip=flip, stem=stem, row_perm=row_perm, label='prep.' + key)
        self.W[key] = out
        return out

    def _block_weights(self, pre, C):
        if pre + 'w49' in self.W:
            return
        P = self.P
        w49 = self.buf('w.' + pre + 'w49', (49, C), torch.float32)
        self.prep.transpose_f32(P[pre + self.NAMES['dw'] + 'weight'], w49, C, 49, label='prep.' + pre + 'w49')
        self.W[pre + 'w49'] = w49
        self._w_plain(pre + self.NAMES['fc1'] + 'weight', 4 * C, C, 1, 1, cs=P[pre + 'norm.weight'])
        b1e = self.buf('w.' + pre + 'b1e', (4 * C,), torch.float32)
        self.prep.bias_fold(P[pre + self.NAMES['fc1'] + 'weight'], P[pre + self.NAMES['fc1'] + 'bias'], None, P[pre + 'norm.bias'], b1e, 4 * C, C)
        self.W[pre + 'b1e'] = b1e
        self._w_plain(pre + self.NAMES['fc2'] + 'weight', C, 4 * C, 1, 1, rs=P[pre + 'gamma'])
        b2e = self.buf('w.' + pre + 'b2e', (C,), torch.float32)
        self.prep.bias_fold(None, P[pre + self.NAMES['fc2'] + 'bias'], P[pre + 'gamma'], None, b2e, C, 4 * C)
        self.W[pre + 'b2e'] = b2e

    def _block_fwd(self, pre, x, res, C):
        assert C % 8 == 0
        F, dt, B = self.fwd, self.dt, self.B
        M = B * res * res
        self._block_weights(pre, C)
        W = self.W
        u = self.tmp('u', (M, C))
        xn = self.blk_act(pre + 'xn', (M, C))
        rstd = self.blk_act(pre + 'rstd', (M,), torch.float32)
        fused = self._mlp_fused(C)
        a = None if fused else self.blk_act(pre + 'a', (M, 4 * C))
        g = self.buf(pre + 'g', (M, 4 * C)) if (self.training and not fused) else None
        y = self.buf(pre + 'y', (M, C))
        dp = self.dp_scale.get(pre)
        cur = F.lane
        for lane, r0, r1, b0, b1 in (self._fsplits(res * res) if cur == 0 else [(cur, 0, M, 0, B)]):
            F.lane = lane
            F.dwconv7_fwd(x[r0:r1], W[pre + 'w49'], self.P[pre + self.NAMES['dw'] + 'bias'], u[r0:r1], b1 - b0, res, res, C, dt,
                          label=pre + 'dw')
            F.layernorm_fwd(u[r0:r1], None, None, xn[r0:r1], None, rstd[r0:r1], r1 - r0, C, 1e-6, dt, label=pre + 'ln')
            if fused:
                F.mlp_fwd(xn[r0:r1], W[pre + self.NAMES['fc1'] + 'weight'], W[pre + 'b1e'], W[pre + self.NAMES['fc2'] + 'weight'],
                          W[pre + 'b2e'], y[r0:r1], r1 - r0, C, dt, R=x[r0:r1], rowscale=dp[b0:b1] if dp is not None else None,
                          rows_per_scale=res * res, label=pre + 'mlp')
                continue
            F.gemm(xn[r0:r1], W[pre + self.NAMES['fc1'] + 'weight'], a[r0:r1], r1 - r0, 4 * C, C, dt, bias=W[pre + 'b1e'], act=ACT_GELU,
                   C2=g[r0:r1] if g is not None else None, c2_mode=2 if g is not None else 0, label=pre + 'fc1')
            F.gemm(a[r0:r1], W[pre + self.NAMES['fc2'] + 'weight'], y[r0:r1], r1 - r0, C, 4 * C, dt, bias=W[pre + 'b2e'],
                   rowscale=dp[b0:b1] if dp is not None else None, rows_per_scale=res * res, R=x[r0:r1], ldr=C,
                   label=pre + 'fc2')
        F.lane = cur
        self.blocks[pre] = dict(x=x, xn=xn, rstd=rstd, a=a, g=g, y=y, res=res, C=C, fused=fused)
        return y

    def _mlp_fused(self, C):
        allowed = [int(v) for v in os.environ.get('GA_FUSED_MLP', '96').split(',') if v.strip()]
        if not self.training and 'GA_FUSED_MLP' not in os.environ:
            allowed.append(192)
        return C in allowed and ops.mlp_supported(C, 4 * C, self.dt)

    def _block_bwd(self, pre, dy, dx, next_pre=None):
        Bk, dt, B, P, W = self.bwd, self.dt, self.B, self.P, self.W
        b = self.blocks[pre]
        res, C = b['res'], b['C']
        M = B * res * res
        dp = self.dp_scale.get(pre)
        dyz = dy
        par, dz_tag = '', 'dyz'
        if self.async_wgrad and Bk.lane == 0:
            self._bwd_seq += 1
            par = str(self._bwd_seq & 1)
            dz_tag = f'dyz{self._bwd_seq % 3}'
            Bk.join_async(f'blk{self._bwd_seq - 2}')
        if dp is not None:
            if pre in self._pre_dyz:
                dyz = self._pre_dyz.pop(pre)
            else:
                dyz = self.tmp(dz_tag, (M, C))
                Bk.rowscale(dy, dp, dyz, M * C, res * res * C, dt, label=pre + 'dp')
        side = self.async_wgrad and Bk.lane == 0
        wl = ASYNC_LANE if side else Bk.lane
        ml = Bk.lane
        G2, gb2 = self.gbuf((C, 4 * C)), self.gbuf((C,))
        gb1 = self.gbuf((4 * C,))
        G1 = self.gbuf((4 * C, C))
        g = self.tmp('g', (M, C))
        if b['fused'] and self.mlp_wg1 and ops.mlp_bwd_wgrad_supported(C, 4 * C, dt):
            a = self.tmp('a' + par, (M, 4 * C))
            part = self.tmp('mlpwg' + par, (ops.mlp_bwd_partials(M, C, dt) // 4,), torch.float32)
            Bk.mlp_bwd(b['xn'], dyz, W[pre + self.NAMES['fc1'] + 'weight'], W[pre + 'b1e'], W[pre + self.NAMES['fc2'] + 'weight.T'],
                       W[pre + self.NAMES['fc1'] + 'weight.T'], a, None, g, M, C, dt, dW1=G1, db1=gb1, partials=part, label=pre + 'mlpb')
            Bk.lane = wl
            Bk.wgrad(dyz, a, G2, M, C, 4 * C, dt, dbias=gb2, label=pre + 'wg2')
            Bk.lane = ml
        elif b['fused']:
            a = self.tmp('a' + par, (M, 4 * C))
            dh = self.tmp('dh' + par, (M, 4 * C))
            Bk.mlp_bwd(b['xn'], dyz, W[pre + self.NAMES['fc1'] + 'weight'], W[pre + 'b1e'], W[pre + self.NAMES['fc2'] + 'weight.T'],
                       W[pre + self.NAMES['fc1'] + 'weight.T'], a, dh, g, M, C, dt, label=pre + 'mlpb')
            Bk.lane = wl
            Bk.wgrad(dyz, a, G2, M, C, 4 * C, dt, dbias=gb2, label=pre + 'wg2')
            Bk.wgrad(dh, b['xn'], G1, M, 4 * C, C, dt, dbias=gb1, label=pre + 'wg1')
            Bk.lane = ml
        else:
            dh = self.tmp('dh' + par, (M, 4 * C))
            Bk.lane = wl
            Bk.wgrad(dyz, b['a'], G2, M, C, 4 * C, dt, dbias=gb2, label=pre + 'wg2')
            Bk.lane = ml
            Bk.gemm(dyz, W[pre + self.NAMES['fc2'] + 'weight.T'], dh, M, 4 * C, C, dt, H=b['g'], ldh=4 * C, h_is_deriv=True, colsum=gb1,
                    label=pre + 'dg2')
            Bk.lane = wl
            Bk.wgrad(dh, b['xn'], G1, M, 4 * C, C, dt, label=pre + 'wg1')
            Bk.lane = ml
            Bk.gemm(dh, W[pre + self.NAMES['fc1'] + 'weight.T'], g, M, C, 4 * C, dt, label=pre + 'dg1')
        du = self.tmp('du' + par, (M, C))
        Bk.layernorm_bwd(g, b['xn'], None, b['rstd'], None, None, du, None, None, M, C, True, dt, label=pre + 'lnb')
        dw49 = self.gbuf((49, C))
        Bk.lane = wl
        Bk.dwconv7_bwd_weight(du, b['x'], dw49, self.grad(pre + self.NAMES['dw'] + 'bias'), B, res, res, C, dt, label=pre + 'dww')
        Bk.lane = ml
        if side:
            Bk.async_mark(f'blk{self._bwd_seq}')
        dx2 = dp_next = None
        if next_pre is not None and self.fuse_dp:
            dp_next = self.dp_scale.get(next_pre)
            if dp_next is not None:
                nxt = f'dyz{(self._bwd_seq + 1) % 3}' if side else 'dyz'
                dx2 = self._pre_dyz[next_pre] = self.tmp(nxt, (M, C))
        Bk.dwconv7_bwd_data(du, W[pre + 'w49'], dy, dx, B, res, res, C, dt, dx2=dx2, scale2=dp_next, label=pre + 'dwd')
        Bk.weight_unfold(G2, 4 * C, C, 4 * C, gb=gb2, W=P[pre + self.NAMES['fc2'] + 'weight'], b=P[pre + self.NAMES['fc2'] + 'bias'],
                         rs=P[pre + 'gamma'], dW=self.grad(pre + self.NAMES['fc2'] + 'weight'), db=self.grad(pre + self.NAMES['fc2'] + 'bias'),
                         d_rs=self.grad(pre + 'gamma'), label=pre + 'unf2')
        Bk.weight_unfold(G1, C, 4 * C, C, gb=gb1, W=P[pre + self.NAMES['fc1'] + 'weight'], b=P[pre + self.NAMES['fc1'] + 'bias'],
                         cs=P[pre + 'norm.weight'], v=P[pre + 'norm.bias'], dW=self.grad(pre + self.NAMES['fc1'] + 'weight'),
                         db=self.grad(pre + self.NAMES['fc1'] + 'bias'), d_cs=self.grad(pre + 'norm.weight'),
                         d_v=self.grad(pre + 'norm.bias'), label=pre + 'unf1')
        Bk.transpose_f32(dw49, self.grad(pre + self.NAMES['dw'] + 'weight'), 49, C, accumulate=True, label=pre + 'unfdw')

    def _bn_pool(self, C):
        off = (self.bn_pool_off + 63) // 64 * 64
        assert off + C <= self.bn_pool.numel()
        self.bn_pool_off = off + C
        return self.bn_pool[off:off + C]

    def _bn_bufs(self, pre, C, zero=False):
        return dict(s=self._bn_pool(C), q=self._bn_pool(C),
                    mean=self.buf(pre + 'bmean', (C,), torch.float32, zero=zero), rstd=self.buf(pre + 'brstd', (C,), torch.float32, zero=zero),
                    scale=self.buf(pre + 'scale', (C,), torch.float32, zero=zero), shift=self.buf(pre + 'shift', (C,), torch.float32, zero=zero))

    def _sync_allreduce(self, plan, t, label):
        c = self.sync_bn
        plan._add('ga_allreduce_bucket', (c.handle, ops._ptr(t), t.numel(), GA_F32, 1.0, None, 0), label, keep=(t, c))

    def _bn_finalize(self, pre, bn, n, C):
        if self.sync_bn is not None and self.training:
            self._sync_allreduce(self.fwd, bn['s'], pre + 'sync.s')
            self._sync_allreduce(self.fwd, bn['q'], pre + 'sync.q')
            n = n * self.sync_bn.world
        self.fwd.bn_finalize(bn['s'], bn['q'], n, self.P[pre + 'weight'], self.P[pre + 'bias'], 1e-5, 0.1,
                             self.Bf[pre + 'running_mean'], self.Bf[pre + 'running_var'], bn['mean'], bn['rstd'],
                             bn['scale'], bn['shift'], C, self.training, label=pre + 'fin')

    def _bn_bwd(self, pre, bn, dy, y_relu, x, dx, rows, C, rowscale=None, rps=1, ldx=0, lddx=0, weight=None, c_real=None):
        Bk = self.bwd
        s1, s2 = self.gbuf((C,)), self.gbuf((C,))
        Bk.bn_bwd_reduce(dy, y_relu, x, bn['mean'], bn['rstd'], s1, s2, rows, C, self.dt, rowscale=rowscale,
                         rows_per_scale=rps, ldx=ldx, label=pre + 'bnr')
        n = rows
        if self.sync_bn is not None:
            Bk._add('ga_axpy_f32', (ops._ptr(self.grad(pre + 'weight')), ops._ptr(s2), 1.0, c_real or C), pre + 'dgamma', keep=(s2,))
            Bk._add('ga_axpy_f32', (ops._ptr(self.grad(pre + 'bias')), ops._ptr(s1), 1.0, c_real or C), pre + 'dbeta', keep=(s1,))
            self._sync_allreduce(Bk, s1, pre + 'sync.s1')
            self._sync_allreduce(Bk, s2, pre + 'sync.s2')
            n = rows * self.sync_bn.world
        Bk.bn_bwd_apply(dy, y_relu, x, bn['mean'], bn['rstd'], self.P[pre + 'weight'] if weight is None else weight, s1, s2, n, dx,
                        rows, C, self.dt, rowscale=rowscale, rows_per_scale=rps, ldx=ldx, lddx=lddx, label=pre + 'bna')
        if self.sync_bn is None:
            Bk.axpy_f32(self.grad(pre + 'weight'), s2, 1.0, c_real or C)
            Bk.axpy_f32(self.grad(pre + 'bias'), s1, 1.0, c_real or C)

    def _bott_pad(self, pre, w, wp, ctot, cout):
        P = self.P
        R = P[pre + 'se.fc1.weight'].shape[0]
        spec = {'conv1.weight': ((wp, ctot), w, ctot, ctot, ctot), 'conv2.weight': ((wp, wp, 3, 3), w, 9 * w, 9 * w, 9 * wp),
                'conv3.weight': ((cout, wp), cout, w, w, wp), 'se.fc1.weight': ((R, wp), R, w, w, wp),
                'se.fc2.weight': ((wp, R), w, R, R, R), 'se.fc2.bias': ((wp,), 1, w, w, wp)}
        for bn in ('bn1', 'bn2'):
            spec[bn + '.weight'] = ((wp,), 1, w, w, wp)
            spec[bn + '.bias'] = ((wp,), 1, w, w, wp)
        PB, back = {}, []
        for name, (shape, rows, cols, lds, ldd) in spec.items():
            buf = self.buf('pad.' + pre + name, shape, torch.float32, zero=True)
            self.prep.pad_copy_f32(P[pre + name], buf, rows, cols, lds, ldd, label='prep.pad.' + pre + name)
            PB[pre + name] = buf
            back.append((name, rows, cols, lds, ldd))
        return PB, back

    def _bottleneck_fwd(self, cat, M4, ctot, cout):
        F, dt, B, P, T = self.fwd, self.dt, self.B, self.P, self.training
        pre = self.bott_prefix
        w_real = cout // 4
        w = pad8(w_real)
        HW = M4 // B
        st = self.bott = dict(cat=cat, w=w, w_real=w_real, cout=cout, ctot=ctot, PB=None)
        if w != w_real:
            st['PB'], st['back'] = self._bott_pad(pre, w_real, w, ctot, cout)
            P = dict(P)
            P.update(st['PB'])
        st['P'] = P
        stats = T

        def conv_bn(name, bnname, A, Wt, N, Kdim, bias=None, n_real=None, **kw):
            c = self.act(pre + name + '.out', (M4, N))
            bn = self._bn_bufs(pre + bnname + '.', N, zero=bool(n_real) and n_real != N)
            F.gemm(A, Wt, c, M4, N, Kdim, dt, bias=bias, colsum=bn['s'] if stats else None,
                   colsumsq=bn['q'] if stats else None, label=pre + name, **kw)
            self._bn_finalize(pre + bnname + '.', bn, M4, n_real or N)
            return c, bn

        F.lane = ASYNC_LANE if self.par_branch else 0
        Wds = self._w_plain(pre + 'downsample.0.weight', cout, ctot, 1, 1)
        st['sc'], st['bnd'] = conv_bn('downsample.0', 'downsample.1', cat, Wds, cout, ctot, bias=P[pre + 'downsample.0.bias'])
        t = self.tmp('bott.t', (M4, cout))
        F.affine_act(st['sc'], st['bnd']['scale'], st['bnd']['shift'], None, t, M4, cout, False, dt, label=pre + 'bnd')
        F.lane = 0
        Wc1 = self._w_plain(pre + 'conv1.weight', w, ctot, 1, 1, src=P[pre + 'conv1.weight'])
        st['c1'], st['bn1'] = conv_bn('conv1', 'bn1', cat, Wc1, w, ctot, n_real=w_real)
        st['y1'] = self.act(pre + 'y1', (M4, w))
        F.affine_act(st['c1'], st['bn1']['scale'], st['bn1']['shift'], None, st['y1'], M4, w, True, dt, label=pre + 'bn1')
        Wc2 = self._w_plain(pre + 'conv2.weight', w, w, 3, 3, flip=True, src=P[pre + 'conv2.weight'])
        st['c2'], st['bn2'] = conv_bn('conv2', 'bn2', st['y1'], Wc2, w, 9 * w, n_real=w_real, a_kind=A_CONV3, a_dims=(14, 14, w))
        st['y2'] = self.act(pre + 'y2', (M4, w))
        F.affine_act(st['c2'], st['bn2']['scale'], st['bn2']['shift'], None, st['y2'], M4, w, True, dt, label=pre + 'bn2')
        R = P[pre + 'se.fc1.weight'].shape[0]
        st['R'] = R
        st['sp'] = self.act(pre + 'se.sp', (B, w), torch.float32)
        st['hid'] = self.act(pre + 'se.hid', (B, R), torch.float32)
        st['gate'] = self.act(pre + 'se.gate', (B, w), torch.float32)
        F.spatial_sum(st['y2'], None, st['sp'], B, HW, w, 1.0 / HW, dt, label=pre + 'se.pool')
        F.se_mlp_fwd(st['sp'], P[pre + 'se.fc1.weight'], P[pre + 'se.fc1.bias'], P[pre + 'se.fc2.weight'],
                     P[pre + 'se.fc2.bias'], st['hid'], st['gate'], B, w, R, label=pre + 'se.mlp')
        st['z'] = self.act(pre + 'se.z', (M4, w))
        F.chan_scale(st['y2'], st['gate'], None, st['z'], B, HW, w, dt, label=pre + 'se.scale')
        Wc3 = self._w_plain(pre + 'conv3.weight', cout, w, 1, 1, src=P[pre + 'conv3.weight'])
        st['c3'], st['bn3'] = conv_bn('conv3', 'bn3', st['z'], Wc3, cout, w)
        x4 = self.buf(pre + 'out', (M4, cout))
        if self.par_branch:
            F.join_async()
        F.affine_act(st['c3'], st['bn3']['scale'], st['bn3']['shift'], t, x4, M4, cout, True, dt,
                     rowscale=self.dp_scale.get(pre), rows_per_scale=HW, label=pre + 'bn3+add')
        st['x4'] = x4
        return x4

    def _bottleneck_bwd(self, dx4, dcat):
        Bk, dt, B, P, W = self.bwd, self.dt, self.B, self.bott['P'], self.W
        pre = self.bott_prefix
        st = self.bott
        w, cout, ctot = st['w'], st['cout'], st['ctot']
        padded = st['PB'] is not None
        GB = {pre + name: self.gbuf(tuple(st['PB'][pre + name].shape)) for name, *_ in st['back']} if padded else {}

        def grad(name):
            return GB[name] if name in GB else self.grad(name)

        M4 = dx4.shape[0]
        HW = M4 // B
        dp = self.dp_scale.get(pre)
        dc3 = self.tmp('bott.dc3', (M4, cout))
        self._bn_bwd(pre + 'bn3.', st['bn3'], dx4, st['x4'], st['c3'], dc3, M4, cout, rowscale=dp, rps=HW)
# ... 640 lines not shown
```

imagenet-models_amd/ops.py:

```python
import ctypes as C
import os

import torch

from . import _lib as L
from ._lib import (A_CONV3, A_CONV3S2, A_NEIGH2, A_PATCH2, A_PLAIN, A_STEM4_NCHW, ACT_GELU, ACT_NONE, ACT_RELU, C_PLAIN, C_UNPATCH2,
                   GA_BF16, GA_F32)


def ga_dtype(t):
    if isinstance(t, torch.dtype):
        dt = t
    else:
        dt = t.dtype
    if dt == torch.bfloat16:
        return GA_BF16
    if dt == torch.float32:
        return GA_F32
    raise TypeError(f'unsupported dtype {dt}')


def torch_dtype(ga):
    return torch.bfloat16 if ga == GA_BF16 else torch.float32

# ... 226 lines not shown
                if not used:
                    if apend:
                        ajoin()
                        apend = False
                    fork.record(main)
                if lane not in used:
                    streams[lane - 1].wait_event(fork)
                    used.append(lane)
                rc = fn(*args, streams[lane - 1].cuda_stream)
            if rc != 0:
                L.check(rc, f'{self.name}:{label}')
        for ln in used:
            done[ln - 1].record(streams[ln - 1])
            main.wait_event(done[ln - 1])
        if apend:
            ajoin()

    def __len__(self):
        return len(self.calls)

    def mark(self, name):
        self.marks[name] = len(self.calls)

    def run_range(self, start, end, stream=None):
        self.finalize()
        s = current_stream_ptr() if stream is None else stream
        if any(self.lanes[start:end]):
            return self._run_lanes(start, end)
        for fn, args, label in self.calls[start:end]:
            rc = fn(*args, s)
            if rc != 0:
                L.check(rc, f'{self.name}:{label}')

    def gemm(self, A, B, Cout, M, N, K, dtype, lda=None, ldb=None, ldc=None, batch=1, strideA=0, strideB=0, strideC=0,
             a_batch_mod=0, a_kind=A_PLAIN, a_dims=(0, 0, 0), a_act=ACT_NONE, c_kind=C_PLAIN, c_dims=(0, 0, 0),
             c_f32=False, alpha=1.0, bias=None, strideBias=0, act=ACT_NONE, H=None, ldh=0, strideH=0, rowscale=None,
             rows_per_scale=1, R=None, ldr=0, strideR=0, relu_after=False, colsum=None, colsumsq=None, strideCol=0,
             C2=None, c2_mode=0, h_is_deriv=False, label=None):
        d = L.GemmDesc()
        d.M, d.N, d.K, d.batch, d.dtype = M, N, K, batch, dtype
        d.A, d.lda, d.strideA, d.a_batch_mod, d.a_kind = _ptr(A), (K if lda is None else lda), strideA, a_batch_mod, a_kind
        d.a_H, d.a_W, d.a_C = a_dims
        d.a_act = a_act
        d.B, d.ldb, d.strideB = _ptr(B), (K if ldb is None else ldb), strideB
        d.C, d.ldc, d.strideC, d.c_kind = _ptr(Cout), (N if ldc is None else ldc), strideC, c_kind
        d.c_H, d.c_W, d.c_C = c_dims
        d.c_f32 = int(c_f32)
        d.C2, d.c2_mode = _ptr(C2), c2_mode
        d.h_is_deriv = int(h_is_deriv)
        d.alpha = alpha
        d.bias, d.strideBias, d.act = _ptr(bias), strideBias, act
        d.H, d.ldh, d.strideH = _ptr(H), ldh, strideH
        d.rowscale, d.rows_per_scale = _ptr(rowscale), rows_per_scale
        d.R, d.ldr, d.strideR, d.relu_after = _ptr(R), ldr, strideR, int(relu_after)
        d.colsum, d.colsumsq, d.strideCol = _ptr(colsum), _ptr(colsumsq), strideCol
        self._add('ga_gemm', (C.byref(d),), label, keep=(d, A, B, Cout, bias, H, rowscale, R, colsum, colsumsq, C2))

    def attn_desc(self, qkv, out, lse, B, N, H, hd, scale, dtype, ldq=None, ldo=None):
        d = L.AttnDesc()
        d.B, d.N, d.H, d.hd, d.scale, d.dtype = B, N, H, hd, scale, dtype
        d.qkv, d.ldq, d.out, d.ldo, d.lse = _ptr(qkv), (3 * H * hd if ldq is None else ldq), _ptr(out), (H * hd if ldo is None else ldo), _ptr(lse)
        self.keep.extend([d, qkv, out, lse])
        return d

    def attn_fwd(self, d, label=None):
        self._add('ga_attn_fwd', (C.byref(d),), label, keep=(d,))

    def attn_bwd(self, d, dout, dqkv, ws, label=None):
        self._add('ga_attn_bwd', (C.byref(d), _ptr(dout), _ptr(dqkv), _ptr(ws), ws.numel() * ws.element_size()), label,
                  keep=(d, dout, dqkv, ws))

    def patchify(self, x, out, P, dtype, label=None):
        B, CH, H, W = x.shape
        self._add('ga_patchify', (_ptr(x), _ptr(out), B, CH, H, W, P, dtype), label, keep=(x, out))

    def patchify_strided(self, x, out, P, S, dtype, label=None):
        B, CH, H, W = x.shape
        self._add('ga_patchify_strided', (_ptr(x), _ptr(out), B, CH, H, W, P, S, dtype), label, keep=(x, out))

    def pos_add_fwd(self, tok, pos, x0, B, Np, Cdim, dtype, label=None):
        self._add('ga_pos_add_fwd', (_ptr(tok), _ptr(pos), _ptr(x0), B, Np, Cdim, dtype), label, keep=(tok, pos, x0))

    def pos_add_bwd(self, dx0, dpos, B, Np, Cdim, dtype, label=None):
        self._add('ga_pos_add_bwd', (_ptr(dx0), _ptr(dpos), B, Np, Cdim, dtype), label, keep=(dx0, dpos))

    def dwpool_fwd(self, x, w, bias, y, B, H, W_, Cin, mult, dtype, label=None):
        self._add('ga_dwpool_fwd', (_ptr(x), _ptr(w), _ptr(bias), _ptr(y), B, H, W_, Cin, mult, dtype), label, keep=(x, w, bias, y))

    def dwpool_bwd_data(self, dy, w, dx, B, H, W_, Cin, mult, dtype, label=None):
        self._add('ga_dwpool_bwd_data', (_ptr(dy), _ptr(w), _ptr(dx), B, H, W_, Cin, mult, dtype), label, keep=(dy, w, dx))

    def dwpool_bwd_weight(self, dy, x, dw, db, B, H, W_, Cin, mult, dtype, label=None):
        self._add('ga_dwpool_bwd_weight', (_ptr(dy), _ptr(x), _ptr(dw), _ptr(db), B, H, W_, Cin, mult, dtype), label, keep=(dy, x, dw, db))

    def resize_concat_fwd(self, src, dst, B, Hin, Win, Cdim, Hout, Wout, ldd, c_off, dtype, label=None):
        self._add('ga_resize_concat_fwd', (_ptr(src), _ptr(dst), B, Hin, Win, Cdim, Hout, Wout, ldd, c_off, dtype), label, keep=(src, dst))

    def resize_concat_bwd(self, dcat, dsrc, B, Hin, Win, Cdim, Hout, Wout, ldd, c_off, dtype, label=None):
        self._add('ga_resize_concat_bwd', (_ptr(dcat), _ptr(dsrc), B, Hin, Win, Cdim, Hout, Wout, ldd, c_off, dtype), label, keep=(dcat, dsrc))

    def rows_bcast(self, src, dst, B, HW, Cdim, scale, dtype, label=None):
        self._add('ga_rows_bcast', (_ptr(src), _ptr(dst), B, HW, Cdim, scale, dtype), label, keep=(src, dst))

    def token_gap_fwd(self, x, y, B, N, Cdim, dtype, label=None):
        self._add('ga_token_gap_fwd', (_ptr(x), _ptr(y), B, N, Cdim, dtype), label, keep=(x, y))

    def token_gap_bwd(self, dy, dx, B, N, Cdim, dtype, label=None):
        self._add('ga_token_gap_bwd', (_ptr(dy), _ptr(dx), B, N, Cdim, dtype), label, keep=(dy, dx))

    def vit_embed_fwd(self, tok, cls, pos, x0, B, Np, Cdim, dtype, label=None):
        self._add('ga_vit_embed_fwd', (_ptr(tok), _ptr(cls), _ptr(pos), _ptr(x0), B, Np, Cdim, dtype), label, keep=(tok, cls, pos, x0))

    def vit_embed_bwd(self, dx0, dtok, dcls, dpos, B, Np, Cdim, dtype, label=None):
        self._add('ga_vit_embed_bwd', (_ptr(dx0), _ptr(dtok), _ptr(dcls), _ptr(dpos), B, Np, Cdim, dtype), label, keep=(dx0, dtok, dcls, dpos))

    def small_linear_desc(self, A, W, Y, rows, groups, Ng, Kg, dtype, lda, a_gstride, ldy, bias=None, a_perm=None, col_scale=None,
                          rowscale=None, rows_per_scale=1, R=None, ldr=0, Yraw=None):
        d = L.SmallLinearDesc()
        d.rows, d.groups, d.Ng, d.Kg, d.dtype = rows, groups, Ng, Kg, dtype
        d.A, d.lda, d.a_gstride, d.a_perm = _ptr(A), lda, a_gstride, _ptr(a_perm)
        d.W, d.bias, d.col_scale = _ptr(W), _ptr(bias), _ptr(col_scale)
        d.rowscale, d.rows_per_scale, d.R, d.ldr = _ptr(rowscale), rows_per_scale, _ptr(R), ldr
        d.Y, d.ldy, d.Yraw = _ptr(Y), ldy, _ptr(Yraw)
        self.keep.extend([d, A, W, Y, bias, a_perm, col_scale, rowscale, R, Yraw])
        return d

    def small_linear_fwd(self, d, label=None):
        self._add('ga_small_linear_fwd', (C.byref(d),), label, keep=(d,))

    def small_linear_bwd(self, d, dY, dA=None, accumulate_dA=False, dW=None, dbias=None, dcol_scale=None, label=None):
        self._add('ga_small_linear_bwd', (C.byref(d), _ptr(dY), _ptr(dA), int(accumulate_dA), _ptr(dW), _ptr(dbias), _ptr(dcol_scale)),
                  label, keep=(d, dY, dA, dW, dbias, dcol_scale))

    def colstats(self, x, ld, rows, Cdim, s, q, dtype, label=None):
        self._add('ga_colstats', (_ptr(x), ld, rows, Cdim, _ptr(s), _ptr(q), dtype), label, keep=(x, s, q))

    def pad_copy_f32(self, src, dst, rows, cols, lds, ldd, accumulate=False, label=None):
        self._add('ga_pad_copy_f32', (_ptr(src), _ptr(dst), rows, cols, lds, ldd, int(accumulate)), label, keep=(src, dst))

    def stem4_ln_fwd(self, x, W, ldw, bias, gamma, beta, pre, y, mean, rstd, B, H, W_, Cdim, eps, label=None):
        self._add('ga_stem4_ln_fwd', (_ptr(x), _ptr(W), ldw, _ptr(bias), _ptr(gamma), _ptr(beta), _ptr(pre), _ptr(y), _ptr(mean), _ptr(rstd),
                                      B, H, W_, Cdim, eps), label, keep=(x, W, bias, gamma, beta, pre, y, mean, rstd))

    def blockdiag_f32(self, src, dst, R, rg, ng, cg, ld, to_diag=True, accumulate=False, label=None):
        self._add('ga_blockdiag_f32', (_ptr(src), _ptr(dst), R, rg, ng, cg, ld, int(to_diag), int(accumulate)), label, keep=(src, dst))

    def pad_groups_f32(self, src, dst, R, Cdim, RG, RGp, CG, CGp, unpad=False, accumulate=False, label=None):
        self._add('ga_pad_groups_f32', (_ptr(src), _ptr(dst), R, Cdim, RG, RGp, CG, CGp, int(unpad), int(accumulate)), label,
                  keep=(src, dst))

    def pad_copy(self, src, dst, rows, cols, lds, ldd, dtype, accumulate=False, label=None):
        self._add('ga_pad_copy', (_ptr(src), _ptr(dst), rows, cols, lds, ldd, int(accumulate), dtype), label, keep=(src, dst))

    def mlp_fwd(self, X, W1, b1, W2, b2, Y, M, Cdim, dtype, ldw1=None, ldw2=None, R=None, rowscale=None, rows_per_scale=1, label=None):
        d = L.MlpDesc()
        H = 4 * Cdim
        d.X, d.ldx, d.W1, d.ldw1, d.b1 = _ptr(X), Cdim, _ptr(W1), (Cdim if ldw1 is None else ldw1), _ptr(b1)
        d.W2, d.ldw2, d.b2 = _ptr(W2), (H if ldw2 is None else ldw2), _ptr(b2)
        d.R, d.ldr, d.rowscale, d.rows_per_scale = _ptr(R), Cdim, _ptr(rowscale), rows_per_scale
        d.Y, d.ldy, d.M, d.C, d.H, d.dtype = _ptr(Y), Cdim, M, Cdim, H, dtype
        self._add('ga_mlp_fwd', (C.byref(d),), label, keep=(d, X, W1, b1, W2, b2, R, rowscale, Y))

    def mlp_bwd(self, X, DY, W1, b1, W2T, W1T, A, DH, DX, M, Cdim, dtype, ldw1=None, ldw2t=None, ldw1t=None, label=None,
                dW1=None, db1=None, partials=None, max_blocks=0):
        d = L.MlpBwdDesc()
        H = 4 * Cdim
        d.X, d.ldx, d.DY, d.lddy = _ptr(X), Cdim, _ptr(DY), Cdim
        d.W1, d.ldw1, d.b1 = _ptr(W1), (Cdim if ldw1 is None else ldw1), _ptr(b1)
        d.W2T, d.ldw2t, d.W1T, d.ldw1t = _ptr(W2T), (Cdim if ldw2t is None else ldw2t), _ptr(W1T), (H if ldw1t is None else ldw1t)
        d.A, d.lda, d.DH, d.lddh, d.DX, d.lddx = _ptr(A), H, _ptr(DH), H, _ptr(DX), Cdim
        d.M, d.C, d.H, d.dtype = M, Cdim, H, dtype
        if dW1 is not None:
            assert dW1.dtype == torch.float32 and db1 is not None and db1.dtype == torch.float32 and partials is not None
            assert dW1.stride(-1) == 1 and partials.dtype == torch.float32 and partials.is_contiguous()
            d.dW1, d.ldw, d.db1 = _ptr(dW1), dW1.stride(0), _ptr(db1)
            d.partials, d.partials_bytes, d.max_blocks = _ptr(partials), partials.numel() * 4, max_blocks
        self._add('ga_mlp_bwd', (C.byref(d),), label, keep=(d, X, DY, W1, b1, W2T, W1T, A, DH, DX, dW1, db1, partials))

    def wgrad(self, Y, X, dW, M, N, K, dtype, ldy=None, ldx=None, ldw=None, batch=1, strideY=0, strideX=0, strideW=0,
              x_kind=A_PLAIN, x_dims=(0, 0, 0), x_act=ACT_NONE, dbias=None, strideDbias=0, alpha=1.0, split_m=None,
              accumulate=True, x_batch_mod=0, label=None):
        d = L.WgradDesc()
        d.M, d.N, d.K, d.batch, d.dtype = M, N, K, batch, dtype
        d.Y, d.ldy, d.strideY = _ptr(Y), (N if ldy is None else ldy), strideY
        d.X, d.ldx, d.strideX, d.x_kind = _ptr(X), (K if ldx is None else ldx), strideX, x_kind
        d.x_batch_mod = x_batch_mod
        d.x_H, d.x_W, d.x_C = x_dims
        d.x_act = x_act
        d.dW, d.ldw, d.strideW = _ptr(dW), (K if ldw is None else ldw), strideW
        d.dbias, d.strideDbias = _ptr(dbias), strideDbias
        d.alpha = alpha
        if split_m is None:
            split_m = pick_split_m(M, N, K, batch, dtype)
        d.split_m, d.accumulate = split_m, int(accumulate)
        need = self.lib.ga_wgrad_workspace(C.byref(d))
        if need:
            def patch(ptr, nbytes, d=d):
                d.workspace, d.ws_bytes = ptr, nbytes
            self._want_workspace(int(need), patch)
        self._add('ga_wgrad', (C.byref(d),), label, keep=(d, Y, X, dW, dbias))

    def weight_prep(self, w, G, Co, Ci, KH, KW, dtype, out=None, ldo=0, outT=None, ldt=0, rs=None, cs=None, flip=False,
                    stem=False, row_perm=None, t_cols=0, label=None):
        d = L.WprepDesc()
        d.w, d.G, d.Co, d.Ci, d.KH, d.KW = _ptr(w), G, Co, Ci, KH, KW
        d.rs, d.cs, d.row_perm, d.dtype = _ptr(rs), _ptr(cs), _ptr(row_perm), dtype
        d.out, d.ldo, d.outT, d.ldt, d.flip, d.stem = _ptr(out), ldo, _ptr(outT), ldt, int(flip), int(stem)
        d.t_cols = t_cols
        if self.defer:
            self._pend['wprep'].append(d)
            self.keep.extend((w, out, outT, rs, cs, row_perm))
            return
        self._add('ga_weight_prep', (C.byref(d),), label, keep=(d, w, out, outT, rs, cs, row_perm))

    def bias_fold(self, W, b, rs, v, be, N, Cdim, row_perm=None, label=None):
        if self.defer:
            self._small(kind=2, y=_ptr(be), x=_ptr(W), R=N, C=Cdim, b=_ptr(b), rs=_ptr(rs), v=_ptr(v), row_perm=_ptr(row_perm))
            self.keep.extend((W, b, rs, v, be, row_perm))
            return
        self._add('ga_bias_fold', (_ptr(W), _ptr(b), _ptr(rs), _ptr(v), _ptr(row_perm), _ptr(be), N, Cdim), label,
                  keep=(W, b, rs, v, be, row_perm))

    def weight_unfold(self, G, ldg, N, Ci, KH=1, KW=1, gb=None, W=None, b=None, rs=None, cs=None, v=None, stem=False, dW=None,
                      db=None, d_rs=None, d_cs=None, d_v=None, row_perm=None, label=None):
        d = L.WunfoldDesc()
        d.G, d.ldg, d.gb, d.W, d.b, d.rs, d.cs, d.v = _ptr(G), ldg, _ptr(gb), _ptr(W), _ptr(b), _ptr(rs), _ptr(cs), _ptr(v)
        d.row_perm = _ptr(row_perm)
        d.N, d.Ci, d.KH, d.KW, d.stem = N, Ci, KH, KW, int(stem)
        d.dW, d.db, d.d_rs, d.d_cs, d.d_v = _ptr(dW), _ptr(db), _ptr(d_rs), _ptr(d_cs), _ptr(d_v)
        if self.defer:
            self._pend['unfold'].append(d)
            self.keep.extend((G, gb, W, b, rs, cs, v, dW, db, d_rs, d_cs, d_v, row_perm))
            return
        self._add('ga_weight_unfold', (C.byref(d),), label, keep=(d, G, gb, W, b, rs, cs, v, dW, db, d_rs, d_cs, d_v, row_perm))

    def dwconv7_fwd(self, x, w49, bias, y, B, H, W, Cdim, dtype, label=None):
        self._add('ga_dwconv7_fwd', (_ptr(x), _ptr(w49), _ptr(bias), _ptr(y), B, H, W, Cdim, dtype), label,
                  keep=(x, w49, bias, y))

    def dwconv7_bwd_data(self, dy, w49, res, dx, B, H, W, Cdim, dtype, dx2=None, scale2=None, label=None):
        if dx2 is not None:
            self._add('ga_dwconv7_bwd_data2', (_ptr(dy), _ptr(w49), _ptr(res), _ptr(dx), _ptr(dx2), _ptr(scale2), B, H, W,
                                               Cdim, dtype), label, keep=(dy, w49, res, dx, dx2, scale2))
            return
        self._add('ga_dwconv7_bwd_data', (_ptr(dy), _ptr(w49), _ptr(res), _ptr(dx), B, H, W, Cdim, dtype), label,
                  keep=(dy, w49, res, dx))

    def dwconv7_bwd_weight(self, dy, x, dw49, dbias, B, H, W, Cdim, dtype, label=None):
        need = int(self.lib.ga_dwconv7_bwd_weight_workspace(B, H, W, Cdim, dtype))
        head = (_ptr(dy), _ptr(x), _ptr(dw49), _ptr(dbias), B, H, W, Cdim, dtype)
        box = {}

        def patch(ptr, nbytes):
            box['ws'] = (ptr, nbytes)
            if 'idx' in box:
                fn, _, lb = self.calls[box['idx']]
                self.calls[box['idx']] = (fn, head + (ptr, nbytes), lb)
        self._want_workspace(need, patch)
        self._add('ga_dwconv7_bwd_weight', head + box.get('ws', (None, 0)), label, keep=(dy, x, dw49, dbias))
        box['idx'] = len(self.calls) - 1

    def dwconv3_fwd(self, x, w9, y, B, H, W, Cdim, stride, dtype, colsum=None, colsumsq=None, label=None):
        self._add('ga_dwconv3_fwd', (_ptr(x), _ptr(w9), _ptr(y), B, H, W, Cdim, stride, _ptr(colsum), _ptr(colsumsq), dtype), label,
                  keep=(x, w9, y, colsum, colsumsq))

    def dwconv3_bwd_data(self, dy, w9, dx, B, H, W, Cdim, stride, dtype, label=None):
        self._add('ga_dwconv3_bwd_data', (_ptr(dy), _ptr(w9), _ptr(dx), B, H, W, Cdim, stride, dtype), label, keep=(dy, w9, dx))

    def dwconv3_bwd_weight(self, dy, x, dw9, B, H, W, Cdim, stride, dtype, label=None):
        need = int(self.lib.ga_dwconv3_bwd_weight_workspace(B, H, W, Cdim, stride, dtype))
        head = (_ptr(dy), _ptr(x), _ptr(dw9), B, H, W, Cdim, stride, dtype)
        box = {}

        def patch(ptr, nbytes):
            box['ws'] = (ptr, nbytes)
            if 'idx' in box:
                fn, _, lb = self.calls[box['idx']]
                self.calls[box['idx']] = (fn, head + (ptr, nbytes), lb)
        self._want_workspace(need, patch)
        self._add('ga_dwconv3_bwd_weight', head + box.get('ws', (None, 0)), label, keep=(dy, x, dw9))
        box['idx'] = len(self.calls) - 1

    def maxpool3s2_fwd(self, x, y, idx, B, H, W, Cdim, dtype, label=None):
        self._add('ga_maxpool3s2_fwd', (_ptr(x), _ptr(y), _ptr(idx), B, H, W, Cdim, dtype), label, keep=(x, y, idx))

    def maxpool3s2_bwd(self, dy, idx, dx, B, H, W, Cdim, dtype, accumulate=False, label=None):
        self._add('ga_maxpool3s2_bwd', (_ptr(dy), _ptr(idx), _ptr(dx), B, H, W, Cdim, int(accumulate), dtype), label, keep=(dy, idx, dx))

    def bn_gelu_fwd(self, x, scale, shift, y, rows, Cdim, dtype, label=None):
        self._add('ga_bn_gelu_fwd', (_ptr(x), _ptr(scale), _ptr(shift), _ptr(y), rows, Cdim, dtype), label, keep=(x, scale, shift, y))

    def bn_gelu_bwd_reduce(self, dy, x, scale, shift, mean, rstd, s1, s2, rows, Cdim, dtype, label=None):
        need = int(self.lib.ga_bn_gelu_bwd_workspace(rows, Cdim))
        head = (_ptr(dy), _ptr(x), _ptr(scale), _ptr(shift), _ptr(mean), _ptr(rstd), _ptr(s1), _ptr(s2), rows, Cdim, dtype)
        box = {}

        def patch(ptr, nbytes):
            box['ws'] = (ptr, nbytes)
            if 'idx' in box:
                fn, _, lb = self.calls[box['idx']]
                self.calls[box['idx']] = (fn, head + (ptr, nbytes), lb)
        self._want_workspace(need, patch)
        self._add('ga_bn_gelu_bwd_reduce', head + box.get('ws', (None, 0)), label, keep=(dy, x, scale, shift, mean, rstd, s1, s2))
        box['idx'] = len(self.calls) - 1

    def bn_gelu_bwd_apply(self, dy, x, scale, shift, mean, rstd, w, s1, s2, n, dx, rows, Cdim, dtype, label=None):
        self._add('ga_bn_gelu_bwd_apply', (_ptr(dy), _ptr(x), _ptr(scale), _ptr(shift), _ptr(mean), _ptr(rstd), _ptr(w), _ptr(s1), _ptr(s2), n,
                                           _ptr(dx), rows, Cdim, dtype), label, keep=(dy, x, scale, shift, mean, rstd, w, s1, s2, dx))

    def se_bn_fwd(self, S, HW, scale3, shift3, W1, g1, b1, rmean, rvar, W2, b2, hpre, mean, rstd, h, gate, B, Cdim, R, training, label=None):
        args = (S, scale3, shift3, W1, g1, b1, rmean, rvar, W2, b2, hpre, mean, rstd, h, gate)
        self._add('ga_se_bn_fwd', (_ptr(S), HW) + tuple(_ptr(t) for t in args[1:]) + (B, Cdim, R, int(training)), label, keep=args)

    def se_bn_bwd(self, P1, P2, rowscale, g3, b3, mean3, rstd3, S, HW, scale3, shift3, W1, g1, b1, W2, hpre, mean, rstd, h, gate, dz, dhpre,
                  ds, s1, s2, dW1, dg1, db1, dW2, db2, B, Cdim, R, label=None):
        pre = (P1, P2, rowscale, g3, b3, mean3, rstd3, S)
        post = (scale3, shift3, W1, g1, b1, W2, hpre, mean, rstd, h, gate, dz, dhpre, ds, s1, s2, dW1, dg1, db1, dW2, db2)
        self._add('ga_se_bn_bwd', tuple(_ptr(t) for t in pre) + (HW,) + tuple(_ptr(t) for t in post) + (B, Cdim, R), label, keep=pre + post)

    def se_residual_fwd(self, x3, scale3, shift3, gate, rowscale, res, rscale, rshift, y, B, HW, Cdim, dtype, label=None):
        args = (x3, scale3, shift3, gate, rowscale, res, rscale, rshift, y)
        self._add('ga_se_residual_fwd', tuple(_ptr(t) for t in args) + (B, HW, Cdim, dtype), label, keep=args)

    def se_residual_bwd_a(self, dy, y, x3, mean3, rstd3, dm, P1, P2, B, HW, Cdim, dtype, label=None):
        args = (dy, y, x3, mean3, rstd3, dm, P1, P2)
        self._add('ga_se_residual_bwd_a', tuple(_ptr(t) for t in args) + (B, HW, Cdim, dtype), label, keep=args)

    def se_residual_bwd_b(self, dm, x3, mean3, rstd3, g3, gate, rowscale, ds, s1, s2, dx3, B, HW, Cdim, dtype, label=None):
        args = (dm, x3, mean3, rstd3, g3, gate, rowscale, ds, s1, s2, dx3)
        self._add('ga_se_residual_bwd_b', tuple(_ptr(t) for t in args) + (B, HW, Cdim, dtype), label, keep=args)
# ... 169 lines not shown

    def map_tokens_fwd(self, e, tok, B, Cdim, T, add_mean, dtype, label=None):
        self._add('ga_map_tokens_fwd', (_ptr(e), _ptr(tok), B, Cdim, T, int(add_mean), dtype), label, keep=(e, tok))

    def map_tokens_bwd(self, dtok, de, B, Cdim, T, add_mean, dtype, label=None):
        self._add('ga_map_tokens_bwd', (_ptr(dtok), _ptr(de), B, Cdim, T, int(add_mean), dtype), label, keep=(dtok, de))

    def class_attn_mt_fwd(self, q, kv_cls, kv_tok, tok_ld, out, P, mask, B, T, N, heads, hd, scale, dtype, label=None):
        self._add('ga_class_attn_mt_fwd', (_ptr(q), _ptr(kv_cls), _ptr(kv_tok), tok_ld, _ptr(out), _ptr(P), _ptr(mask), B, T, N, heads,
                                           hd, scale, dtype), label, keep=(q, kv_cls, kv_tok, out, P, mask))

    def class_attn_mt_bwd(self, dout, q, kv_cls, kv_tok, tok_ld, P, mask, dq, dkv_cls, dkv_tok, dtok_ld, B, T, N, heads, hd, scale,
                          dtype, label=None):
        self._add('ga_class_attn_mt_bwd', (_ptr(dout), _ptr(q), _ptr(kv_cls), _ptr(kv_tok), tok_ld, _ptr(P), _ptr(mask), _ptr(dq),
                                           _ptr(dkv_cls), _ptr(dkv_tok), dtok_ld, B, T, N, heads, hd, scale, dtype), label,
                  keep=(dout, q, kv_cls, kv_tok, P, mask, dq, dkv_cls, dkv_tok))

    def class_attn_mt_ia_fwd(self, q, kv_cls, kv_tok, tok_ld, out, P, mask, W1, b1, W2, b2, B, T, N, heads, hd, scale, dtype, label=None):
        self._add('ga_class_attn_mt_ia_fwd', (_ptr(q), _ptr(kv_cls), _ptr(kv_tok), tok_ld, _ptr(out), _ptr(P), _ptr(mask), _ptr(W1), _ptr(b1),
                                              _ptr(W2), _ptr(b2), B, T, N, heads, hd, scale, dtype), label,
                  keep=(q, kv_cls, kv_tok, out, P, mask, W1, b1, W2, b2))

    def class_attn_mt_ia_bwd(self, dout, q, kv_cls, kv_tok, tok_ld, P, mask, W1, W2, b2, dq, dkv_cls, dkv_tok, dtok_ld, dW1, db1, dW2, db2,
                             B, T, N, heads, hd, scale, dtype, label=None):
        self._add('ga_class_attn_mt_ia_bwd', (_ptr(dout), _ptr(q), _ptr(kv_cls), _ptr(kv_tok), tok_ld, _ptr(P), _ptr(mask), _ptr(W1), _ptr(W2),
                                              _ptr(b2), _ptr(dq), _ptr(dkv_cls), _ptr(dkv_tok), dtok_ld, _ptr(dW1), _ptr(db1), _ptr(dW2),
                                              _ptr(db2), B, T, N, heads, hd, scale, dtype), label,
                  keep=(dout, q, kv_cls, kv_tok, P, mask, W1, W2, b2, dq, dkv_cls, dkv_tok, dW1, db1, dW2, db2))

    def map_loss_fwd_bwd(self, org, avg, target, loss, dorg, davg, K, B, NC, lam, kind, smoothing, grad_scale, dtype, label=None):
        self._add('ga_map_loss_fwd_bwd', (_ptr(org), _ptr(avg), _ptr(target), _ptr(loss), _ptr(dorg), _ptr(davg), K, B, NC, lam, kind,
                                          smoothing, grad_scale, dtype), label, keep=(org, avg, target, loss, dorg, davg))

    def loss_dense_fwd_bwd(self, org, avg, target, dense, loss, dorg, davg, K, B, NC, lam, kind, smoothing, bce_threshold, grad_scale,
                           dtype, label=None):
        self._add('ga_loss_dense_fwd_bwd', (_ptr(org), _ptr(avg), _ptr(target), _ptr(dense), _ptr(loss), _ptr(dorg), _ptr(davg), K, B, NC,
                                            lam, kind, smoothing, bce_threshold, grad_scale, dtype), label,
                  keep=(org, avg, target, dense, loss, dorg, davg))

    def u8_normalize(self, x, out, mean, std, label=None):
        B, CH, H, W = x.shape
        m = (C.c_float * CH)(*[float(v) for v in mean])
        s = (C.c_float * CH)(*[float(v) for v in std])
        self._add('ga_u8_normalize', (_ptr(x), _ptr(out), B, CH, H, W, m, s), label, keep=(x, out, m, s))

    def input_erase(self, x, out, boxes, max_count, mode, seed, offset, mean=None, std=None, label=None):
        B, CH, H, W = x.shape
        u8 = x.dtype == torch.uint8
        m = (C.c_float * CH)(*[float(v) for v in mean]) if u8 else None
        s = (C.c_float * CH)(*[float(v) for v in std]) if u8 else None
        mask = (1 << 64) - 1
        self._add('ga_input_erase', (_ptr(x), int(u8), _ptr(out), B, CH, H, W, m, s, _ptr(boxes), int(max_count), int(mode),
                                     int(seed) & mask, int(offset) & mask), label, keep=(x, out, boxes, m, s))

    def mixup_batch(self, x, out, lam, cutmix=False, box=(0, 0, 0, 0), label=None):
        B, CH, H, W = x.shape
        yl, yh, xl, xh = (int(v) for v in box)
        self._add('ga_mixup_batch', (_ptr(x), _ptr(out), B, CH, H, W, float(lam), int(cutmix), yl, yh, xl, xh), label, keep=(x, out))

    def mixup_target(self, target, out, NC, lam, smoothing, label=None):
        self._add('ga_mixup_target', (_ptr(target), _ptr(out), target.numel(), NC, float(lam), float(smoothing)), label, keep=(target, out))

    def agc_clip(self, params, grads, units, nunits, clip_factor, eps=1e-3, label=None):
        self._add('ga_agc_clip', (_ptr(params), _ptr(grads), _ptr(units), nunits, float(clip_factor), float(eps)), label,
                  keep=(params, grads, units))

    def gelu_fwd(self, x, y, n, dtype, label=None):
        self._add('ga_gelu_fwd', (_ptr(x), _ptr(y), n, dtype), label, keep=(x, y))

    def gelu_bwd(self, dy, x, dx, n, dtype, label=None):
        self._add('ga_gelu_bwd', (_ptr(dy), _ptr(x), _ptr(dx), n, dtype), label, keep=(dy, x, dx))

    def relu_drop(self, a, mask, out, deriv, n, dtype, label=None):
        self._add('ga_relu_drop', (_ptr(a), _ptr(mask), _ptr(out), _ptr(deriv), n, dtype), label, keep=(a, mask, out, deriv))

    def mask_mul(self, x, mask, res, y, n, dtype, label=None):
        self._add('ga_mask_mul', (_ptr(x), _ptr(mask), _ptr(res), _ptr(y), n, dtype), label, keep=(x, mask, res, y))

    def copy2d(self, src, lds, dst, ldd, rows, cols, dtype, accumulate=False, label=None):
        self._add('ga_copy2d', (_ptr(src), lds, _ptr(dst), ldd, rows, cols, int(accumulate), dtype), label, keep=(src, dst))

    def loss_fwd_bwd(self, logits, target, loss, dlogits, K, B, NC, lam, kind, smoothing, grad_scale, dtype, label=None):
        self._add('ga_loss_fwd_bwd', (_ptr(logits), _ptr(target), _ptr(loss), _ptr(dlogits), K, B, NC, lam, kind,
                                      smoothing, grad_scale, dtype), label, keep=(logits, target, loss, dlogits))

    def heads_topk(self, logits, K, B, NC, topk, out_sum, out_idx, label=None):
        self._add('ga_heads_topk', (_ptr(logits), K, B, NC, topk, _ptr(out_sum), _ptr(out_idx)), label,
                  keep=(logits, out_sum, out_idx))

    def sgd_step(self, p, g, buf, hp, n, nesterov, wd_mult, label=None):
        self._add('ga_sgd_step', (_ptr(p), _ptr(g), _ptr(buf), _ptr(hp), n, int(nesterov), wd_mult), label,
                  keep=(p, g, buf, hp))

    def adamw_step(self, p, g, m, v, hp, n, wd_mult, label=None):
        self._add('ga_adamw_step', (_ptr(p), _ptr(g), _ptr(m), _ptr(v), _ptr(hp), n, wd_mult), label,
                  keep=(p, g, m, v, hp))

    def drop_path_sample(self, out, keep, sites, B, seed, counter, label=None):
        self._add('ga_drop_path_sample', (_ptr(out), _ptr(keep), sites, B, int(seed) & ((1 << 64) - 1), _ptr(counter)), label,
                  keep=(out, keep, counter))

    def dropout_mask_sample(self, out, n, keep, seed, counter, label=None):
        self._add('ga_dropout_mask_sample', (_ptr(out), n, float(keep), int(seed) & ((1 << 64) - 1), _ptr(counter)), label,
                  keep=(out, counter))

    def transpose_f32(self, src, dst, R, Cdim, accumulate=False, label=None):
        if self.defer:
            self._small(kind=1, y=_ptr(dst), x=_ptr(src), R=R, C=Cdim, accumulate=int(accumulate))
            self.keep.extend((src, dst))
            return
        self._add('ga_transpose_f32', (_ptr(src), _ptr(dst), R, Cdim, int(accumulate)), label, keep=(src, dst))

    def axpy_f32(self, y, x, a, n, label=None):
        if self.defer:
            self._small(kind=0, y=_ptr(y), x=_ptr(x), a=a, n=n)
            self.keep.extend((y, x))
            return
        self._add('ga_axpy_f32', (_ptr(y), _ptr(x), a, n), label, keep=(y, x))

    def lamb_stage1(self, p, g, m, v, u, hp, gsumsq, chunks, nchunks, norms, label=None):
        self._add('ga_lamb_stage1', (_ptr(p), _ptr(g), _ptr(m), _ptr(v), _ptr(u), _ptr(hp), _ptr(gsumsq), _ptr(chunks), nchunks,
                                     _ptr(norms)), label, keep=(p, g, m, v, u, hp, gsumsq, chunks, norms))

    def lamb_stage2(self, p, u, hp, chunks, nchunks, norms, label=None):
        self._add('ga_lamb_stage2', (_ptr(p), _ptr(u), _ptr(hp), _ptr(chunks), nchunks, _ptr(norms)), label,
                  keep=(p, u, hp, chunks, norms))

    def lerp_f32(self, y, x, w, n, label=None):
        self._add('ga_lerp_f32', (_ptr(y), _ptr(x), float(w), n), label, keep=(y, x))

    def sumsq_f32(self, x, n, out, label=None):
        self._add('ga_sumsq_f32', (_ptr(x), n, _ptr(out)), label, keep=(x, out))

    def clip_grad_f32(self, g, n, sumsq, limit, mode, label=None):
        self._add('ga_clip_grad_f32', (_ptr(g), n, _ptr(sumsq), float(limit), int(mode)), label, keep=(g, sumsq))

    def rowscale(self, x, s, y, n, elems_per_scale, dtype, label=None):
        self._add('ga_rowscale', (_ptr(x), _ptr(s), _ptr(y), n, elems_per_scale, dtype), label, keep=(x, s, y))

    def cast_from_f32(self, src, dst, n, dtype, label=None):
        self._add('ga_cast_from_f32', (_ptr(src), _ptr(dst), n, dtype), label, keep=(src, dst))

    def cast_to_f32(self, src, dst, n, dtype, label=None):
        self._add('ga_cast_to_f32', (_ptr(src), _ptr(dst), n, dtype), label, keep=(src, dst))

    def zero(self, t, label=None):
        self._add('ga_memset', (_ptr(t), 0, t.numel() * t.element_size()), label or 'zero', keep=(t,))


def mlp_supported(Cdim, H, dtype):
    return bool(L.load().ga_mlp_supported(Cdim, H, dtype))


def mlp_bwd_wgrad_supported(Cdim, H, dtype):
    return bool(L.load().ga_mlp_bwd_wgrad_supported(Cdim, H, dtype))


def mlp_bwd_partials(M, Cdim, dtype, max_blocks=0):
    d = L.MlpBwdDesc()
    d.M, d.C, d.H, d.dtype, d.max_blocks = M, Cdim, 4 * Cdim, dtype, max_blocks
    return int(L.load().ga_mlp_bwd_partials(C.byref(d)))


def cswin_attn_bwd_workspace(d):
    return int(L.load().ga_cswin_attn_bwd_workspace(C.byref(d)))


def zero_(t):
    L.check(L.load().ga_memset(_ptr(t), 0, t.numel() * t.element_size(), current_stream_ptr()), 'ga_memset')
    return t


_NUM_CU = None


def num_cus():
    global _NUM_CU
    if _NUM_CU is None:
        n = C.c_int(256)
        L.check(L.load().ga_device_info(C.byref(n), None, None), 'ga_device_info')
        _NUM_CU = n.value
    return _NUM_CU


def pick_split_m(M, N, K, batch, dtype):
    slab = 64 if dtype == GA_BF16 else 32
    tiles = ((N + 127) // 128) * ((K + 127) // 128) * batch
    want = max(1, (2 * 256) // tiles)
    return int(max(1, min(want, (M + 4 * slab - 1) // (4 * slab))))
```

include/gaext.h:

```cpp
#ifndef GAEXT_H
#define GAEXT_H
#include <stddef.h>
#include <stdint.h>

#ifdef __cplusplus
extern "C" {
#endif

typedef void* ga_stream_t;

enum { GA_F32 = 0, GA_BF16 = 1 };
enum { GA_OK = 0, GA_ERR_BAD_ARG = -1, GA_ERR_UNSUPPORTED = -2, GA_ERR_HIP = -3 };

enum { GA_ACT_NONE = 0, GA_ACT_GELU = 1, GA_ACT_RELU = 2 };

enum {
    GA_A_PLAIN = 0,
    GA_A_PATCH2 = 1,
    GA_A_STEM4_NCHW = 2,
    GA_A_CONV3 = 3,
    GA_A_CONV3S2 = 4,
    GA_A_NEIGH2 = 5
};
enum {
// ... 159 lines not shown
                   float* scale, float* shift, int C, int training, ga_stream_t stream);
int ga_affine_act(const void* x, const float* scale, const float* shift, const void* res, const float* rowscale,
                  int64_t rows_per_scale, void* y, int64_t rows, int C, int relu, int dtype, int64_t ldx, ga_stream_t stream);
int ga_bn_bwd_reduce(const void* dy, const void* y_relu, const void* x, const float* mean, const float* rstd,
                     const float* rowscale, int64_t rows_per_scale, float* s1, float* s2, int64_t rows, int C, int dtype,
                     int64_t ldx, ga_stream_t stream);
int ga_bn_bwd_apply(const void* dy, const void* y_relu, const void* x, const float* mean, const float* rstd,
                    const float* w, const float* s1, const float* s2, const float* rowscale, int64_t rows_per_scale,
                    int64_t n, void* dx, int64_t rows, int C, int dtype, int64_t ldx, int64_t lddx, ga_stream_t stream);

int ga_pool_concat_fwd(const void* src, void* dst, int B, int Hin, int Win, int C, int Hout, int Wout, int ldd,
                       int c_off, int mode, int dtype, ga_stream_t stream);
int ga_pool_concat_bwd(const void* dcat, const void* dres, void* dsrc, int B, int Hin, int Win, int C, int Hout,
                       int Wout, int ldd, int c_off, int mode, int dtype, ga_stream_t stream);

int ga_spatial_sum(const void* a, const void* b2, float* out, int B, int HW, int C, float scale, int dtype,
                   ga_stream_t stream);
int ga_se_mlp_fwd(const float* s, const float* W1, const float* b1, const float* W2, const float* b2, float* hid,
                  float* gate, int B, int C, int R, ga_stream_t stream);
int ga_se_mlp_bwd(const float* dgate, const float* gate, const float* hid, const float* s, const float* W1,
                  const float* W2, float* ds, float ds_scale, float* dW1, float* db1, float* dW2, float* db2, int B,
                  int C, int R, ga_stream_t stream);
int ga_chan_scale(const void* x, const float* g, const float* add, void* y, int B, int HW, int C, int dtype,
                  ga_stream_t stream);

int ga_gram_pack_fwd(const float* G, void* out, float* inv_norm, int B, int C, int groups, int Kp, int dtype,
                     ga_stream_t stream);
int ga_gram_pack_bwd(const void* dvec, const void* vhat, const float* inv_norm, void* S, int B, int C, int groups,
                     int Kp, int dtype, ga_stream_t stream);

size_t ga_gram_f64_fwd_workspace(int B, int C);
size_t ga_gram_f64_bwd_workspace(int B, int C);
int ga_gram_f64_fwd(const void* x, void* vec, double* inv_norm, double* G64, size_t g64_bytes, int B, int HW, int C, int H,
                    int groups, int Kp, int dtype, ga_stream_t stream);
int ga_gram_f64_bwd(const void* dvec, const void* x, const double* G64, const double* inv_norm, void* dx, void* workspace,
                    size_t ws_bytes, int B, int HW, int C, int H, int groups, int Kp, int dtype, ga_stream_t stream);

int ga_token_cat(const void* cls, const void* tok, void* u, int B, int N, int C, int dtype, ga_stream_t stream);
int ga_token_split(const void* du, void* dcls, void* dtok, int B, int N, int C, int acc_cls, int acc_tok, int dtype,
                   ga_stream_t stream);
int ga_class_attn_fwd(const void* q, const void* kv, void* out, float* P, int B, int N, int heads, int hd, float scale,
                      int dtype, ga_stream_t stream);
int ga_class_attn_bwd(const void* dout, const void* q, const void* kv, const float* P, void* dq, void* dkv, int B, int N,
                      int heads, int hd, float scale, int dtype, ga_stream_t stream);
int ga_class_attn_fwd2(const void* q, const void* kv_cls, const void* kv_tok, int64_t tok_ld, void* out, float* P, int B, int N,
                       int heads, int hd, float scale, int dtype, ga_stream_t stream);
int ga_class_attn_bwd2(const void* dout, const void* q, const void* kv_cls, const void* kv_tok, int64_t tok_ld, const float* P,
                       void* dq, void* dkv_cls, void* dkv_tok, int B, int N, int heads, int hd, float scale, int dtype,
                       ga_stream_t stream);

int ga_loss_fwd_bwd(const float* logits, const int64_t* target, float* loss, void* dlogits, int K, int B, int NC,
                    float lam, int kind, float smoothing, float grad_scale, int dtype, ga_stream_t stream);
int ga_heads_topk(const float* logits, int K, int B, int NC, int topk, float* out_sum, int64_t* out_idx,
                  ga_stream_t stream);

int ga_sgd_step(float* p, const float* g, float* buf, const float* hp, int64_t n, int nesterov, float wd_mult,
                ga_stream_t stream);
int ga_adamw_step(float* p, const float* g, float* m, float* v, const float* hp, int64_t n, float wd_mult,
                  ga_stream_t stream);

typedef struct {
    int kind;
    float* y; const float* x; float a; int64_t n;
    int R, C, accumulate;
    const float* b; const float* rs; const float* v; const int* row_perm;
} ga_small_desc;
int ga_weight_prep_batch(const ga_wprep_desc* jobs_dev, int n, ga_stream_t stream);
int ga_weight_unfold_batch(const ga_wunfold_desc* jobs_dev, int n, ga_stream_t stream);
int ga_small_batch(const ga_small_desc* jobs_dev, int n, ga_stream_t stream);

int ga_lamb_stage1(const float* p, const float* g, float* m, float* v, float* u, const float* hp, const float* gsumsq,
                   const int* chunks, int nchunks, float* norms, ga_stream_t stream);
int ga_lamb_stage2(float* p, const float* u, const float* hp, const int* chunks, int nchunks, const float* norms,
                   ga_stream_t stream);

int ga_sumsq_f32(const float* x, int64_t n, float* out, ga_stream_t stream);
int ga_clip_grad_f32(float* g, int64_t n, const float* sumsq, float limit, int mode, ga_stream_t stream);

typedef struct {
    int B, reso, C, heads, nbranch;
    int Hs[2], Ws[2];
    const float* lepe_w[2];
    const float* lepe_b[2];
    float scale;
    int dtype;
    const void* qkv; int64_t ldq;
    void* out; int64_t ldo;
} ga_cswin_attn_desc;
int ga_cswin_attn_fwd(const ga_cswin_attn_desc* d, ga_stream_t stream);
size_t ga_cswin_attn_bwd_workspace(const ga_cswin_attn_desc* d);
int ga_cswin_attn_bwd(const ga_cswin_attn_desc* d, const void* dout, void* dqkv, void* lepe_ws, size_t ws_bytes, ga_stream_t stream);
int ga_cswin_lepe_wgrad_reduce(const ga_cswin_attn_desc* d, const void* lepe_ws, float* dw0, float* db0, float* dw1, float* db1,
                               ga_stream_t stream);
int ga_cswin_lepe_wgrad(const ga_cswin_attn_desc* d, const void* dout, float* dw0, float* db0, float* dw1, float* db1,
                        ga_stream_t stream);
int ga_layernorm_gelu_fwd(const void* x, const float* w, const float* b, void* y, float* mean, float* rstd, int64_t rows,
                          int C, float eps, int dtype, ga_stream_t stream);
int ga_layernorm_gelu_bwd(const void* g, const void* x, const float* mean, const float* rstd, const float* w, const float* b,
                          void* dx, float* dw, float* db, int64_t rows, int C, int dtype, ga_stream_t stream);
int ga_nchw3_to_nhwc8(const float* x, void* y, int B, int H, int W, int dtype, ga_stream_t stream);
int ga_convw_pack(const float* w, void* out, int Co, int Ci, int taps, int Cp, int64_t ldo, int dtype, ga_stream_t stream);
int ga_convw_unpack_grad(const float* G, float* dW, int Co, int Ci, int taps, int Cp, int64_t ldg, ga_stream_t stream);
int ga_conv3s2_dgrad_prep(const float* w, void* out, int Co, int Ci, int64_t ldo, int dtype, ga_stream_t stream);

int ga_gram_pack_fwd2(const float* G, void* out, float* inv_norm, int B, int C, int groups, int Kp, int ntok, int dtype,
                      ga_stream_t stream);
int ga_gram_pack_bwd2(const void* dvec, const void* vhat, const float* inv_norm, void* S, int B, int C, int groups, int Kp,
                      int ntok, int dtype, ga_stream_t stream);
int ga_map_tokens_fwd(const void* e, void* tok, int B, int C, int T, int add_mean, int dtype, ga_stream_t stream);
int ga_map_tokens_bwd(const void* dtok, void* de, int B, int C, int T, int add_mean, int dtype, ga_stream_t stream);
int ga_class_attn_mt_fwd(const void* q, const void* kv_cls, const void* kv_tok, int64_t tok_ld, void* out, float* P,
                         const float* mask, int B, int T, int N, int heads, int hd, float scale, int dtype, ga_stream_t stream);
int ga_class_attn_mt_bwd(const void* dout, const void* q, const void* kv_cls, const void* kv_tok, int64_t tok_ld, const float* P,
                         const float* mask, void* dq, void* dkv_cls, void* dkv_tok, int64_t dtok_ld, int B, int T, int N,
                         int heads, int hd, float scale, int dtype, ga_stream_t stream);
int ga_class_attn_mt_ia_fwd(const void* q, const void* kv_cls, const void* kv_tok, int64_t tok_ld, void* out, float* P,
                            const float* mask, const float* W1, const float* b1, const float* W2, const float* b2, int B, int T, int N,
                            int heads, int hd, float scale, int dtype, ga_stream_t stream);
int ga_class_attn_mt_ia_bwd(const void* dout, const void* q, const void* kv_cls, const void* kv_tok, int64_t tok_ld, const float* P,
                            const float* mask, const float* W1, const float* W2, const float* b2, void* dq, void* dkv_cls,
                            void* dkv_tok, int64_t dtok_ld, float* dW1, float* db1, float* dW2, float* db2, int B, int T, int N,
                            int heads, int hd, float scale, int dtype, ga_stream_t stream);
int ga_map_loss_fwd_bwd(const float* org, const float* avg, const int64_t* target, float* loss, void* dorg, void* davg, int K,
                        int B, int NC, float lam, int kind, float smoothing, float grad_scale, int dtype, ga_stream_t stream);
int ga_loss_dense_fwd_bwd(const float* org, const float* avg, const int64_t* target, const float* dense, float* loss, void* dorg,
                          void* davg, int K, int B, int NC, float lam, int kind, float smoothing, float bce_threshold,
                          float grad_scale, int dtype, ga_stream_t stream);
int ga_mixup_batch(const float* x, float* out, int B, int CH, int H, int W, double lam, int cutmix, int yl, int yh, int xl, int xh,
                   ga_stream_t stream);
int ga_mixup_target(const int64_t* target, float* out, int B, int NC, double lam, double smoothing, ga_stream_t stream);
int ga_u8_normalize(const void* x, float* out, int B, int CH, int H, int W, const float* mean, const float* std, ga_stream_t stream);
int ga_input_erase(const void* x, int x_is_u8, float* out, int B, int CH, int H, int W, const float* mean, const float* std,
                   const int32_t* boxes, int max_count, int mode, uint64_t seed, uint64_t offset, ga_stream_t stream);
int ga_agc_clip(const float* params, float* grads, const int64_t* units, int nunits, float clip_factor, float eps, ga_stream_t stream);
int ga_gelu_fwd(const void* x, void* y, int64_t n, int dtype, ga_stream_t stream);
int ga_gelu_bwd(const void* dy, const void* x, void* dx, int64_t n, int dtype, ga_stream_t stream);
int ga_relu_drop(const void* a, const float* mask, void* out, void* deriv, int64_t n, int dtype, ga_stream_t stream);
int ga_mask_mul(const void* x, const float* mask, const void* res, void* y, int64_t n, int dtype, ga_stream_t stream);
int ga_copy2d(const void* src, int64_t lds, void* dst, int64_t ldd, int64_t rows, int cols, int accumulate, int dtype,
              ga_stream_t stream);

int ga_drop_path_sample(float* out, const float* keep, int sites, int B, uint64_t seed, uint64_t* counter, ga_stream_t stream);

int ga_dropout_mask_sample(float* out, int64_t n, float keep, uint64_t seed, uint64_t* counter, ga_stream_t stream);

typedef struct {
    const void* X; int64_t ldx;
    const void* W1; int64_t ldw1; const float* b1;
    const void* W2; int64_t ldw2; const float* b2;
    const void* R; int64_t ldr;
    const float* rowscale; int rows_per_scale;
    void* Y; int64_t ldy;
    int64_t M; int C, H, dtype;
} ga_mlp_desc;
typedef struct {
    const void* X; int64_t ldx;
    const void* DY; int64_t lddy;
    const void* W1; int64_t ldw1; const float* b1;
    const void* W2T; int64_t ldw2t;
    const void* W1T; int64_t ldw1t;
    void* A; int64_t lda;
    void* DH; int64_t lddh;
    void* DX; int64_t lddx;
    int64_t M; int C, H, dtype;
    float* dW1; int64_t ldw;
    float* db1;
    float* partials; size_t partials_bytes;
    int max_blocks;
} ga_mlp_bwd_desc;
int ga_mlp_supported(int C, int H, int dtype);
int ga_mlp_fwd(const ga_mlp_desc* d, ga_stream_t stream);
int ga_mlp_bwd(const ga_mlp_bwd_desc* d, ga_stream_t stream);
int ga_mlp_bwd_wgrad_supported(int C, int H, int dtype);
size_t ga_mlp_bwd_partials(const ga_mlp_bwd_desc* d);

typedef struct {
    int rows, groups, Ng, Kg;
    const void* A; int64_t lda; int64_t a_gstride; const int* a_perm;
    const float* W; const float* bias; const float* col_scale;
    const float* rowscale; int rows_per_scale;
    const void* R; int64_t ldr;
    void* Y; int64_t ldy; void* Yraw;
    int dtype;
} ga_small_linear_desc;
int ga_small_linear_fwd(const ga_small_linear_desc* d, ga_stream_t stream);
int ga_small_linear_bwd(const ga_small_linear_desc* d, const void* dY, void* dA, int accumulate_dA, float* dW, float* dbias,
                        float* dcol_scale, ga_stream_t stream);
int ga_colstats(const void* x, int64_t ld, int rows, int C, float* sum, float* sumsq, int dtype, ga_stream_t stream);
int ga_pad_copy_f32(const float* src, float* dst, int64_t rows, int64_t cols, int64_t lds, int64_t ldd, int accumulate, ga_stream_t stream);
int ga_stem4_ln_fwd(const float* x, const void* W, int64_t ldw, const float* bias, const float* gamma, const float* beta, void* pre,
                    void* y, float* mean, float* rstd, int B, int H, int W_, int C, float eps, ga_stream_t stream);
int ga_blockdiag_f32(const float* src, float* dst, int64_t R, int rg, int ng, int cg, int64_t ld, int to_diag, int accumulate,
                     ga_stream_t stream);
int ga_pad_groups_f32(const float* src, float* dst, int64_t R, int64_t C, int RG, int RGp, int CG, int CGp, int unpad, int accumulate,
                      ga_stream_t stream);
int ga_pad_copy(const void* src, void* dst, int64_t rows, int64_t cols, int64_t lds, int64_t ldd, int accumulate, int dtype,
                ga_stream_t stream);

typedef struct {
    int B, N, H, hd;
    float scale;
    int dtype;
    const void* qkv; int64_t ldq;
    void* out; int64_t ldo;
    float* lse;
} ga_attn_desc;
int ga_attn_fwd(const ga_attn_desc* d, ga_stream_t stream);
size_t ga_attn_bwd_workspace(const ga_attn_desc* d);
int ga_attn_bwd(const ga_attn_desc* d, const void* dout, void* dqkv, void* workspace, size_t ws_bytes, ga_stream_t stream);
int ga_patchify(const float* x, void* out, int B, int CH, int H, int W, int P, int dtype, ga_stream_t stream);
int ga_vit_embed_fwd(const void* tok, const float* cls, const float* pos, void* x0, int B, int Np, int C, int dtype, ga_stream_t stream);
int ga_vit_embed_bwd(const void* dx0, void* dtok, float* dcls, float* dpos, int B, int Np, int C, int dtype, ga_stream_t stream);

int ga_patchify_strided(const float* x, void* out, int B, int CH, int H, int W, int P, int S, int dtype, ga_stream_t stream);
int ga_pos_add_fwd(const void* tok, const float* pos, void* x0, int B, int Np, int C, int dtype, ga_stream_t stream);
int ga_pos_add_bwd(const void* dx0, float* dpos, int B, int Np, int C, int dtype, ga_stream_t stream);
int ga_dwpool_fwd(const void* x, const float* w, const float* bias, void* y, int B, int H, int W, int Cin, int mult, int dtype,
                  ga_stream_t stream);
int ga_dwpool_bwd_data(const void* dy, const float* w, void* dx, int B, int H, int W, int Cin, int mult, int dtype, ga_stream_t stream);
int ga_dwpool_bwd_weight(const void* dy, const void* x, float* dw, float* db, int B, int H, int W, int Cin, int mult, int dtype,
                         ga_stream_t stream);
int ga_resize_concat_fwd(const void* src, void* dst, int B, int Hin, int Win, int C, int Hout, int Wout, int64_t ldd, int c_off,
                         int dtype, ga_stream_t stream);
int ga_resize_concat_bwd(const void* dcat, void* dsrc, int B, int Hin, int Win, int C, int Hout, int Wout, int64_t ldd, int c_off,
                         int dtype, ga_stream_t stream);
int ga_rows_bcast(const void* src, void* dst, int B, int HW, int C, float scale, int dtype, ga_stream_t stream);
int ga_token_gap_fwd(const void* x, void* y, int B, int N, int C, int dtype, ga_stream_t stream);
int ga_token_gap_bwd(const void* dy, void* dx, int B, int N, int C, int dtype, ga_stream_t stream);

int ga_memset(void* p, int value, size_t bytes, ga_stream_t stream);
int ga_transpose_f32(const float* in, float* out, int R, int C, int accumulate, ga_stream_t stream);
int ga_axpy_f32(float* y, const float* x, float a, int64_t n, ga_stream_t stream);
int ga_lerp_f32(float* y, const float* x, float w, int64_t n, ga_stream_t stream);
int ga_rowscale(const void* x, const float* s, void* y, int64_t n, int64_t elems_per_scale, int dtype,
                ga_stream_t stream);
int ga_cast_from_f32(const float* src, void* dst, int64_t n, int dtype, ga_stream_t stream);
int ga_cast_to_f32(const void* src, float* dst, int64_t n, int dtype, ga_stream_t stream);

typedef struct ga_comm* ga_comm_t;
int ga_comm_unique_id(void* id128);
int ga_comm_init(ga_comm_t* comm, int rank, int world, const void* id128);
int ga_comm_destroy(ga_comm_t comm);
int ga_comm_info(ga_comm_t comm, int* rank, int* world);
size_t ga_allreduce_workspace(int64_t n, int wire_dtype);
int ga_allreduce_bucket(ga_comm_t comm, float* grads, int64_t n, int wire_dtype, float scale, void* workspace, size_t ws_bytes,
                        ga_stream_t stream);
int ga_reduce_scatter_bucket(ga_comm_t comm, const float* grads, float* shard, int64_t n_per_rank, float scale, ga_stream_t stream);
int ga_allgather_bucket(ga_comm_t comm, const float* shard, float* full, int64_t n_per_rank, ga_stream_t stream);
int ga_comm_broadcast(ga_comm_t comm, void* buf, int64_t n_f32, int root, ga_stream_t stream);

#ifdef __cplusplus
}
#endif
#endif
```

Baseline: 11080 images/sec.

## Fuse LayerNorm into fused MLP forward and backward kernels at C=96

Folds the ConvNeXt block's LayerNorm into the fused MLP kernel for the C=96 stage. The forward normalizes rows while staging them into LDS and writes xn and rstd as side outputs. The backward applies the LayerNorm backward in the dx epilogue and writes du directly. This removes a separate layernorm forward and backward launch per block, plus the round trip of g through global memory. In exchange it adds register pressure and per-row reductions inside the MLP kernels, and reuses LDS for epilogue staging.

```diff
diff --git a/imagenet-models_amd/_lib.py b/imagenet-models_amd/_lib.py
--- a/imagenet-models_amd/_lib.py
+++ b/imagenet-models_amd/_lib.py
@@ -70,14 +70,16 @@
 class MlpDesc(C.Structure):
     _fields_ = [('X', vp), ('ldx', i64), ('W1', vp), ('ldw1', i64), ('b1', vp), ('W2', vp), ('ldw2', i64), ('b2', vp),
                 ('R', vp), ('ldr', i64), ('rowscale', vp), ('rows_per_scale', i32), ('Y', vp), ('ldy', i64),
-                ('M', i64), ('C', i32), ('H', i32), ('dtype', i32)]
+                ('M', i64), ('C', i32), ('H', i32), ('dtype', i32),
+                ('eps', f32), ('XN', vp), ('ldxn', i64), ('RSTD', vp)]
 
 
 class MlpBwdDesc(C.Structure):
     _fields_ = [('X', vp), ('ldx', i64), ('DY', vp), ('lddy', i64), ('W1', vp), ('ldw1', i64), ('b1', vp),
                 ('W2T', vp), ('ldw2t', i64), ('W1T', vp), ('ldw1t', i64), ('A', vp), ('lda', i64), ('DH', vp), ('lddh', i64),
                 ('DX', vp), ('lddx', i64), ('M', i64), ('C', i32), ('H', i32), ('dtype', i32),
-                ('dW1', vp), ('ldw', i64), ('db1', vp), ('partials', vp), ('partials_bytes', C.c_size_t), ('max_blocks', i32)]
+                ('dW1', vp), ('ldw', i64), ('db1', vp), ('partials', vp), ('partials_bytes', C.c_size_t), ('max_blocks', i32),
+                ('RSTD', vp), ('DU', vp), ('lddu', i64)]
 
 
 class SmallLinearDesc(C.Structure):
@@ -228,6 +230,7 @@
     'ga_token_gap_fwd': ([vp, vp, i32, i32, i32, i32, vp], i32),
     'ga_token_gap_bwd': ([vp, vp, i32, i32, i32, i32, vp], i32),
     'ga_mlp_supported': ([i32, i32, i32], i32),
+    'ga_mlp_ln_supported': ([i32, i32, i32], i32),
     'ga_mlp_fwd': ([C.POINTER(MlpDesc), vp], i32),
     'ga_mlp_bwd': ([C.POINTER(MlpBwdDesc), vp], i32),
     'ga_mlp_bwd_wgrad_supported': ([i32, i32, i32], i32),
diff --git a/imagenet-models_amd/csrc/mlp.hip b/imagenet-models_amd/csrc/mlp.hip
--- a/imagenet-models_amd/csrc/mlp.hip
+++ b/imagenet-models_amd/csrc/mlp.hip
@@ -31,6 +31,71 @@
         const int idx = tid + NTHR * i;
         const int r = idx / CPR, c = idx - r * CPR;
         *reinterpret_cast<u32x4_t*>(dst + (c >> 2) * ROWS * 64 + slab_off(r, c & 3)) = v[i];
+    }
+}
+
+template <int C, int NTHR>
+__device__ __forceinline__ void stage_rows_ln(unsigned char* dst, const bf16_t* src, long ld, long row0, long limit, float eps,
+                                              bf16_t* xn, long ldxn, float* rstd, int tid) {
+#pragma clang fp contract(off)
+    constexpr int G = 16, NCH = C / 8, RPP = NTHR / G, NP = BM / RPP;
+    static_assert(NCH <= G && BM % RPP == 0, "one chunk per lane, whole passes");
+    const int lg = tid % G, rib = tid / G;
+    const bool act = lg < NCH;
+    const float invC = 1.f / (float)C;
+    u32x4_t v[NP];
+#pragma unroll
+    for (int i = 0; i < NP; ++i) {
+        const int r = rib + RPP * i;
+        v[i] = u32x4_t{0, 0, 0, 0};
+        if (act && row0 + r < limit) v[i] = __builtin_nontemporal_load(reinterpret_cast<const u32x4_t*>(src + (row0 + r) * ld + lg * 8));
+    }
+    float f[NP][8], mu[NP], rs[NP];
+#pragma unroll
+    for (int i = 0; i < NP; ++i) {
+        unpack8(make_uint4(v[i].x, v[i].y, v[i].z, v[i].w), f[i]);
+        float s = 0.f;
+#pragma unroll
+        for (int e = 0; e < 8; ++e) s += f[i][e];
+        mu[i] = s;
+    }
+#pragma unroll
+    for (int o = G / 2; o > 0; o >>= 1)
+#pragma unroll
+        for (int i = 0; i < NP; ++i) mu[i] += __shfl_xor(mu[i], o, 64);
+#pragma unroll
+    for (int i = 0; i < NP; ++i) {
+        mu[i] *= invC;
+        float q = 0.f;
+        if (act) {
+#pragma unroll
+            for (int e = 0; e < 8; ++e) {
+                const float dlt = f[i][e] - mu[i];
+                q += dlt * dlt;
+            }
+        }
+        rs[i] = q;
+    }
+#pragma unroll
+    for (int o = G / 2; o > 0; o >>= 1)
+#pragma unroll
+        for (int i = 0; i < NP; ++i) rs[i] += __shfl_xor(rs[i], o, 64);
+#pragma unroll
+    for (int i = 0; i < NP; ++i) {
+        const int r = rib + RPP * i;
+        const bool live = row0 + r < limit;
+        rs[i] = rsqrtf(fmaf(rs[i], invC, eps));
+#pragma unroll
+        for (int e = 0; e < 8; ++e) f[i][e] = (f[i][e] - mu[i]) * rs[i];
+        uint4 p = make_uint4(0, 0, 0, 0);
+        if (live) {
+            p.x = pack2bf(f[i][0], f[i][1]); p.y = pack2bf(f[i][2], f[i][3]); p.z = pack2bf(f[i][4], f[i][5]); p.w = pack2bf(f[i][6], f[i][7]);
+        }
+        if (act) {
+            *reinterpret_cast<uint4*>(dst + (lg >> 2) * BM * 64 + slab_off(r, lg & 3)) = p;
+            if (live) store16_nt(xn + (row0 + r) * ldxn + lg * 8, p);
+        }
+        if (live && lg == 0) rstd[row0 + r] = rs[i];
     }
 }
 
@@ -105,7 +170,78 @@
     }
 }
 
-template <int C, int HC>
+template <int C, int NTHR, int NWM, int TM>
+__device__ __forceinline__ void store_rows_lnb(float* Cs, float* Ss, const unsigned char* Xs, const f32x4_t (&acc)[C / 32][TM], int wm,
+                                               int wn, int lane, long m0, long M, const float* rstd, bf16_t* DU, long lddu, int tid) {
+    constexpr int LDC = C + 4, P8 = C / 8, RG = NTHR / P8, WROWS = 16 * TM, WPH = 64 / WROWS;
+    constexpr int NR = (64 + RG - 1) / RG;
+    const int c8 = tid % P8, rg = tid / P8;
+    const float invC = 1.f / (float)C;
+    float rsv[NWM / WPH][NR];
+#pragma unroll
+    for (int piece = 0; piece < NWM / WPH; ++piece)
+#pragma unroll
+        for (int it = 0; it < NR; ++it) {
+            const int row = rg + it * RG;
+            const long m = m0 + piece * 64 + row;
+            rsv[piece][it] = (rg < RG && row < 64 && m < M) ? rstd[m] : 0.f;
+        }
+#pragma unroll
+    for (int tm = 0; tm < TM; ++tm) {
+        const int row = wm * WROWS + 16 * tm + (lane & 15);
+        float s1 = 0.f, s2 = 0.f;
+#pragma unroll
+        for (int tn = 0; tn < C / 32; ++tn) {
+            const int col = wn * (C / 2) + 16 * tn + 4 * (lane >> 4);
+            const uint2 q = *reinterpret_cast<const uint2*>(Xs + (col >> 5) * BM * 64 + slab_off(row, (col & 31) >> 3) + (col & 7) * 2);
+            const float x[4] = {__uint_as_float(q.x << 16), __uint_as_float(q.x & 0xffff0000u), __uint_as_float(q.y << 16),
+                                __uint_as_float(q.y & 0xffff0000u)};
+#pragma unroll
+            for (int r = 0; r < 4; ++r) {
+                s1 += acc[tn][tm][r];
+                s2 = fmaf(acc[tn][tm][r], x[r], s2);
+            }
+        }
+        s1 += __shfl_xor(s1, 16, 64);
+        s2 += __shfl_xor(s2, 16, 64);
+        s1 += __shfl_xor(s1, 32, 64);
+        s2 += __shfl_xor(s2, 32, 64);
+        if (lane < 16) *reinterpret_cast<float2*>(Ss + (row * 2 + wn) * 2) = make_float2(s1, s2);
+    }
+#pragma unroll
+    for (int piece = 0; piece < NWM / WPH; ++piece) {
+        if (piece) __syncthreads();
+        if (wm / WPH == piece) {
+#pragma unroll
+            for (int tn = 0; tn < C / 32; ++tn)
+#pragma unroll
+                for (int tm = 0; tm < TM; ++tm) {
+                    const int row = (wm % WPH) * WROWS + 16 * tm + (lane & 15), col = wn * (C / 2) + 16 * tn + 4 * (lane >> 4);
+                    *reinterpret_cast<f32x4_t*>(Cs + row * LDC + col) = acc[tn][tm];
+                }
+        }
+        __syncthreads();
+        if (rg < RG) {
+#pragma unroll
+            for (int it = 0; it < NR; ++it) {
+                const int row = rg + it * RG, prow = piece * 64 + row;
+                const long m = m0 + prow;
+                if (row >= 64 || m >= M) break;
+                const f32x4_t a = *reinterpret_cast<const f32x4_t*>(Cs + row * LDC + c8 * 8);
+                const f32x4_t b = *reinterpret_cast<const f32x4_t*>(Cs + row * LDC + c8 * 8 + 4);
+                const f32x4_t sm = *reinterpret_cast<const f32x4_t*>(Ss + prow * 4);
+                float v[8] = {a[0], a[1], a[2], a[3], b[0], b[1], b[2], b[3]}, x[8];
+                unpack8(*reinterpret_cast<const uint4*>(Xs + (c8 >> 2) * BM * 64 + slab_off(prow, c8 & 3)), x);
+                const float m1 = (sm[0] + sm[2]) * invC, m2 = (sm[1] + sm[3]) * invC, rs = rsv[piece][it];
+#pragma unroll
+                for (int j = 0; j < 8; ++j) v[j] = rs * (v[j] - m1 - x[j] * m2);
+                store8_nt(DU + m * lddu + c8 * 8, v);
+            }
+        }
+    }
+}
+
+template <int C, int HC, bool LN>
 __global__ __launch_bounds__(256, 2) void mlp_fwd_kernel(const ga_mlp_desc d) {
     constexpr int KS1 = C / 32, KS2 = HC / 32, TN1 = HC / 32, TN2 = C / 32;
     constexpr int XS = KS1 * BM * 64, W1S = KS1 * HC * 64, AS = KS2 * BM * 64;
@@ -151,7 +287,11 @@
     };
 
     w_load(0);
-    stage_rows<BM, KS1, 256>(Xs, reinterpret_cast<const bf16_t*>(d.X), d.ldx, m0, d.M, tid);
+    if constexpr (LN)
+        stage_rows_ln<C, 256>(Xs, reinterpret_cast<const bf16_t*>(d.X), d.ldx, m0, d.M, d.eps, reinterpret_cast<bf16_t*>(d.XN), d.ldxn,
+                              d.RSTD, tid);
+    else
+        stage_rows<BM, KS1, 256>(Xs, reinterpret_cast<const bf16_t*>(d.X), d.ldx, m0, d.M, tid);
     for (int i = tid; i < 4 * C; i += 256) B1s[i] = d.b1[i];
     w1_store();
     w2_store();
@@ -240,13 +380,14 @@
     return *reinterpret_cast<const bf16x8_t*>(&v[0]);
 }
 
-template <int C, int HC, bool WG>
+template <int C, int HC, bool WG, bool LN>
 __global__ __launch_bounds__(512, 1) void mlp_bwd_kernel(const ga_mlp_bwd_desc d) {
     constexpr int KS1 = C / 32, KS2 = HC / 32, TN1 = HC / 32, TN2 = C / 32;
     constexpr int XS = KS1 * BM * 64, WS = KS1 * HC * 64, TS = KS2 * BM * 64;
     constexpr int NPC = HC * C / 8, NI = (NPC + 511) / 512;
     constexpr int NCH = 4 * C / HC;
     static_assert(!WG || (HC == 64 && C == 96), "the in-kernel weight gradient is laid out for 4 x 6 tiles over 8 waves");
+    static_assert(!LN || 64 * (C + 4) * 4 + BM * 16 <= 2 * TS, "the LN epilogue stages on DHs + A2s");
     extern __shared__ __attribute__((aligned(16))) unsigned char smem[];
     unsigned char* Xs = smem;
     unsigned char* Ds = Xs + XS;
@@ -463,8 +604,12 @@
             for (int j = 0; j < RowPre<C, 512>::NR; ++j) nopre[i][j] = u32x4_t{0, 0, 0, 0};
         int stid = tid;
         if constexpr (WG) asm volatile("" : "+v"(stid));
-        store_rows<C, 512, 4, 2>(reinterpret_cast<float*>(smem), dx, stid >> 7, (stid >> 6) & 1, stid & 63, m0, d.M, nullptr, nullptr, 1,
-                                 false, nopre, reinterpret_cast<bf16_t*>(d.DX), d.lddx, stid);
+        if constexpr (LN)
+            store_rows_lnb<C, 512, 4, 2>(reinterpret_cast<float*>(DHs), reinterpret_cast<float*>(DHs) + 64 * (C + 4), Xs, dx, stid >> 7,
+                                         (stid >> 6) & 1, stid & 63, m0, d.M, d.RSTD, reinterpret_cast<bf16_t*>(d.DU), d.lddu, stid);
+        else
+            store_rows<C, 512, 4, 2>(reinterpret_cast<float*>(smem), dx, stid >> 7, (stid >> 6) & 1, stid & 63, m0, d.M, nullptr, nullptr,
+                                     1, false, nopre, reinterpret_cast<bf16_t*>(d.DX), d.lddx, stid);
         if (!next_tile) break;
         tile += gridDim.x;
         __syncthreads();
@@ -529,6 +674,8 @@
 
 extern "C" int ga_mlp_supported(int C, int H, int dtype) { return dtype == GA_BF16 && H == 4 * C && (C == 96 || C == 192); }
 
+extern "C" int ga_mlp_ln_supported(int C, int H, int dtype) { return dtype == GA_BF16 && C == 96 && H == 4 * C; }
+
 extern "C" int ga_mlp_fwd(const ga_mlp_desc* d, ga_stream_t stream) {
     GA_REQUIRE(d && d->X && d->W1 && d->b1 && d->W2 && d->Y && d->M > 0, "ga_mlp_fwd: null / empty descriptor");
     GA_REQUIRE(ga_mlp_supported(d->C, d->H, d->dtype), "ga_mlp_fwd: C=%d H=%d dtype=%d has no fused form (ga_mlp_supported)", d->C,
@@ -540,14 +687,25 @@
     GA_REQUIRE(!d->rowscale || d->rows_per_scale > 0, "ga_mlp_fwd: rows_per_scale");
     hipStream_t s = reinterpret_cast<hipStream_t>(stream);
     const unsigned grid = (unsigned)((d->M + BM - 1) / BM);
+    if (d->XN || d->RSTD) {
+        GA_REQUIRE(ga_mlp_ln_supported(d->C, d->H, d->dtype),
+                   "ga_mlp_fwd: the LayerNorm rides in the kernel at C=96 only, not C=%d H=%d dtype=%d (ga_mlp_ln_supported)", d->C, d->H,
+                   d->dtype);
+        GA_REQUIRE(d->XN && d->RSTD && aligned16(d->XN) && d->ldxn % 8 == 0 && d->ldxn >= d->C && d->eps > 0.f,
+                   "ga_mlp_fwd: XN and RSTD go together, XN 16-byte aligned with ldxn >= C in multiples of 8, eps > 0");
+        constexpr int lds = fwd_lds<96, 64>();
+        GA_REQUIRE(set_lds(mlp_fwd_kernel<96, 64, true>, lds), "ga_mlp_fwd: LDS");
+        hipLaunchKernelGGL((mlp_fwd_kernel<96, 64, true>), dim3(grid), dim3(256), lds, s, *d);
+        return ga_check_launch("ga_mlp_fwd");
+    }
     if (d->C == 96) {
         constexpr int lds = fwd_lds<96, 64>();
-        GA_REQUIRE(set_lds(mlp_fwd_kernel<96, 64>, lds), "ga_mlp_fwd: LDS");
-        hipLaunchKernelGGL((mlp_fwd_kernel<96, 64>), dim3(grid), dim3(256), lds, s, *d);
+        GA_REQUIRE(set_lds(mlp_fwd_kernel<96, 64, false>, lds), "ga_mlp_fwd: LDS");
+        hipLaunchKernelGGL((mlp_fwd_kernel<96, 64, false>), dim3(grid), dim3(256), lds, s, *d);
     } else {
         constexpr int lds = fwd_lds<192, 32>();
-        GA_REQUIRE(set_lds(mlp_fwd_kernel<192, 32>, lds), "ga_mlp_fwd: LDS");
-        hipLaunchKernelGGL((mlp_fwd_kernel<192, 32>), dim3(grid), dim3(256), lds, s, *d);
+        GA_REQUIRE(set_lds(mlp_fwd_kernel<192, 32, false>, lds), "ga_mlp_fwd: LDS");
+        hipLaunchKernelGGL((mlp_fwd_kernel<192, 32, false>), dim3(grid), dim3(256), lds, s, *d);
     }
     return ga_check_launch("ga_mlp_fwd");
 }
@@ -568,7 +726,7 @@
 int wg_grid(const ga_mlp_bwd_desc* d) {
     constexpr int lds = bwd_lds<96, 64>();
     static const int resident = [] {
-        auto kern = mlp_bwd_kernel<96, 64, true>;
+        auto kern = mlp_bwd_kernel<96, 64, true, false>;
         if (!set_lds(kern, lds)) return 0;
         int n = 0;
         if (hipOccupancyMaxActiveBlocksPerMultiprocessor(&n, kern, 512, lds) != hipSuccess || n < 1) n = 1;
@@ -587,7 +745,8 @@
 }
 
 extern "C" int ga_mlp_bwd(const ga_mlp_bwd_desc* d, ga_stream_t stream) {
-    GA_REQUIRE(d && d->X && d->DY && d->W1 && d->b1 && d->W2T && d->W1T && d->DX && d->M > 0, "ga_mlp_bwd: null / empty descriptor");
+    GA_REQUIRE(d && d->X && d->DY && d->W1 && d->b1 && d->W2T && d->W1T && (d->DX || d->DU) && d->M > 0,
+               "ga_mlp_bwd: null / empty descriptor");
     GA_REQUIRE(ga_mlp_supported(d->C, d->H, d->dtype), "ga_mlp_bwd: C=%d H=%d dtype=%d has no fused form (ga_mlp_supported)", d->C,
                d->H, d->dtype);
     GA_REQUIRE(aligned16(d->X) && aligned16(d->DY) && aligned16(d->W1) && aligned16(d->W2T) && aligned16(d->W1T) &&
@@ -595,8 +754,16 @@
                    d->lddy % 8 == 0 && d->ldw1 % 8 == 0 && d->ldw2t % 8 == 0 && d->ldw1t % 8 == 0 && (!d->A || d->lda % 8 == 0) &&
                    (!d->DH || d->lddh % 8 == 0) && d->lddx % 8 == 0 && d->ldx >= d->C && d->lddy >= d->C && d->ldw1 >= d->C &&
                    d->ldw2t >= d->C && d->ldw1t >= d->H && (!d->A || d->lda >= d->H) && (!d->DH || d->lddh >= d->H) &&
-                   d->lddx >= d->C,
+                   (!d->DX || d->lddx >= d->C),
                "ga_mlp_bwd: operands must be 16-byte aligned with leading dimensions in multiples of 8");
+    const bool ln = d->DU != nullptr;
+    if (ln || d->RSTD) {
+        GA_REQUIRE(ga_mlp_ln_supported(d->C, d->H, d->dtype),
+                   "ga_mlp_bwd: the LayerNorm backward rides in the kernel at C=96 only, not C=%d H=%d dtype=%d (ga_mlp_ln_supported)",
+                   d->C, d->H, d->dtype);
+        GA_REQUIRE(d->DU && d->RSTD && !d->DX && aligned16(d->DU) && d->lddu % 8 == 0 && d->lddu >= d->C,
+                   "ga_mlp_bwd: DU needs RSTD and replaces DX (DX = NULL); DU 16-byte aligned with lddu >= C in multiples of 8");
+    }
     hipStream_t s = reinterpret_cast<hipStream_t>(stream);
     if (d->dW1) {
         GA_REQUIRE(ga_mlp_bwd_wgrad_supported(d->C, d->H, d->dtype),
@@ -610,20 +777,29 @@
         const int n = d->H * d->C + d->H;
         GA_REQUIRE(d->partials_bytes >= (size_t)grid * n * sizeof(float), "ga_mlp_bwd: partials holds %zu bytes, %zu needed (ga_mlp_bwd_partials)",
                    (size_t)d->partials_bytes, (size_t)grid * n * sizeof(float));
-        hipLaunchKernelGGL((mlp_bwd_kernel<96, 64, true>), dim3(grid), dim3(512), lds, s, *d);
+        if (ln) {
+            GA_REQUIRE(set_lds(mlp_bwd_kernel<96, 64, true, true>, lds), "ga_mlp_bwd: LDS");
+            hipLaunchKernelGGL((mlp_bwd_kernel<96, 64, true, true>), dim3(grid), dim3(512), lds, s, *d);
+        } else {
+            hipLaunchKernelGGL((mlp_bwd_kernel<96, 64, true, false>), dim3(grid), dim3(512), lds, s, *d);
+        }
         hipLaunchKernelGGL(mlp_bwd_wg_reduce_kernel, dim3((n / 4 + 63) / 64), dim3(256), 0, s, d->partials, grid, n, d->H * d->C, d->C,
                            d->dW1, (long)d->ldw, d->db1);
         return ga_check_launch("ga_mlp_bwd");
     }
     const unsigned grid = (unsigned)((d->M + BM - 1) / BM);
-    if (d->C == 96) {
+    if (ln) {
         constexpr int lds = bwd_lds<96, 64>();
-        GA_REQUIRE(set_lds(mlp_bwd_kernel<96, 64, false>, lds), "ga_mlp_bwd: LDS");
-        hipLaunchKernelGGL((mlp_bwd_kernel<96, 64, false>), dim3(grid), dim3(512), lds, s, *d);
+        GA_REQUIRE(set_lds(mlp_bwd_kernel<96, 64, false, true>, lds), "ga_mlp_bwd: LDS");
+        hipLaunchKernelGGL((mlp_bwd_kernel<96, 64, false, true>), dim3(grid), dim3(512), lds, s, *d);
+    } else if (d->C == 96) {
+        constexpr int lds = bwd_lds<96, 64>();
+        GA_REQUIRE(set_lds(mlp_bwd_kernel<96, 64, false, false>, lds), "ga_mlp_bwd: LDS");
+        hipLaunchKernelGGL((mlp_bwd_kernel<96, 64, false, false>), dim3(grid), dim3(512), lds, s, *d);
     } else {
         constexpr int lds = bwd_lds<192, 32>();
-        GA_REQUIRE(set_lds(mlp_bwd_kernel<192, 32, false>, lds), "ga_mlp_bwd: LDS");
-        hipLaunchKernelGGL((mlp_bwd_kernel<192, 32, false>), dim3(grid), dim3(512), lds, s, *d);
+        GA_REQUIRE(set_lds(mlp_bwd_kernel<192, 32, false, false>, lds), "ga_mlp_bwd: LDS");
+        hipLaunchKernelGGL((mlp_bwd_kernel<192, 32, false, false>), dim3(grid), dim3(512), lds, s, *d);
     }
     return ga_check_launch("ga_mlp_bwd");
 }
diff --git a/imagenet-models_amd/engine.py b/imagenet-models_amd/engine.py
--- a/imagenet-models_amd/engine.py
+++ b/imagenet-models_amd/engine.py
@@ -49,6 +49,9 @@
         self.tmps = {}
         self.async_wgrad = os.environ.get('GAEXT_ASYNC_WGRAD', '1') != '0'
         self.mlp_wg1 = os.environ.get('GAEXT_MLP_WG1', '1') != '0'
+        mlp_ln = os.environ.get('GAEXT_MLP_LN', '1')
+        assert mlp_ln in ('0', '1', 'fwd', 'bwd'), f'GAEXT_MLP_LN={mlp_ln!r}: 0, 1, fwd or bwd'
+        self.mlp_ln_fwd, self.mlp_ln_bwd = mlp_ln in ('1', 'fwd'), mlp_ln in ('1', 'bwd')
         self.fwd_split = max(1, int(os.environ.get('GAEXT_FWD_SPLIT', '2')))
         self.par_branch = os.environ.get('GAEXT_PAR_BRANCH', '1') != '0'
         self.fwd_skew = int(os.environ.get('GAEXT_FWD_SKEW', '-1'))
@@ -461,11 +464,17 @@
         g = self.buf(pre + 'g', (M, 4 * C)) if (self.training and not fused) else None
         y = self.buf(pre + 'y', (M, C))
         dp = self.dp_scale.get(pre)
+        ln_in = fused and self.mlp_ln_fwd and ops.mlp_ln_supported(C, 4 * C, dt)
         cur = F.lane
         for lane, r0, r1, b0, b1 in (self._fsplits(res * res) if cur == 0 else [(cur, 0, M, 0, B)]):
             F.lane = lane
             F.dwconv7_fwd(x[r0:r1], W[pre + 'w49'], self.P[pre + self.NAMES['dw'] + 'bias'], u[r0:r1], b1 - b0, res, res, C, dt,
                           label=pre + 'dw')
+            if ln_in:
+                F.mlp_fwd(u[r0:r1], W[pre + self.NAMES['fc1'] + 'weight'], W[pre + 'b1e'], W[pre + self.NAMES['fc2'] + 'weight'],
+                          W[pre + 'b2e'], y[r0:r1], r1 - r0, C, dt, R=x[r0:r1], rowscale=dp[b0:b1] if dp is not None else None,
+                          rows_per_scale=res * res, XN=xn[r0:r1], RSTD=rstd[r0:r1], eps=1e-6, label=pre + 'mlp')
+                continue
             F.layernorm_fwd(u[r0:r1], None, None, xn[r0:r1], None, rstd[r0:r1], r1 - r0, C, 1e-6, dt, label=pre + 'ln')
             if fused:
                 F.mlp_fwd(xn[r0:r1], W[pre + self.NAMES['fc1'] + 'weight'], W[pre + 'b1e'], W[pre + self.NAMES['fc2'] + 'weight'],
@@ -512,12 +521,15 @@
         G2, gb2 = self.gbuf((C, 4 * C)), self.gbuf((C,))
         gb1 = self.gbuf((4 * C,))
         G1 = self.gbuf((4 * C, C))
-        g = self.tmp('g', (M, C))
+        ln_in = b['fused'] and self.mlp_ln_bwd and ops.mlp_ln_supported(C, 4 * C, dt)
+        du = self.tmp('du' + par, (M, C))
+        g = None if ln_in else self.tmp('g', (M, C))
+        lnk = dict(RSTD=b['rstd'], DU=du) if ln_in else {}
         if b['fused'] and self.mlp_wg1 and ops.mlp_bwd_wgrad_supported(C, 4 * C, dt):
             a = self.tmp('a' + par, (M, 4 * C))
             part = self.tmp('mlpwg' + par, (ops.mlp_bwd_partials(M, C, dt) // 4,), torch.float32)
             Bk.mlp_bwd(b['xn'], dyz, W[pre + self.NAMES['fc1'] + 'weight'], W[pre + 'b1e'], W[pre + self.NAMES['fc2'] + 'weight.T'],
-                       W[pre + self.NAMES['fc1'] + 'weight.T'], a, None, g, M, C, dt, dW1=G1, db1=gb1, partials=part, label=pre + 'mlpb')
+                       W[pre + self.NAMES['fc1'] + 'weight.T'], a, None, g, M, C, dt, dW1=G1, db1=gb1, partials=part, label=pre + 'mlpb', **lnk)
             Bk.lane = wl
             Bk.wgrad(dyz, a, G2, M, C, 4 * C, dt, dbias=gb2, label=pre + 'wg2')
             Bk.lane = ml
@@ -525,7 +537,7 @@
             a = self.tmp('a' + par, (M, 4 * C))
             dh = self.tmp('dh' + par, (M, 4 * C))
             Bk.mlp_bwd(b['xn'], dyz, W[pre + self.NAMES['fc1'] + 'weight'], W[pre + 'b1e'], W[pre + self.NAMES['fc2'] + 'weight.T'],
-                       W[pre + self.NAMES['fc1'] + 'weight.T'], a, dh, g, M, C, dt, label=pre + 'mlpb')
+                       W[pre + self.NAMES['fc1'] + 'weight.T'], a, dh, g, M, C, dt, label=pre + 'mlpb', **lnk)
             Bk.lane = wl
             Bk.wgrad(dyz, a, G2, M, C, 4 * C, dt, dbias=gb2, label=pre + 'wg2')
             Bk.wgrad(dh, b['xn'], G1, M, 4 * C, C, dt, dbias=gb1, label=pre + 'wg1')
@@ -541,8 +553,8 @@
             Bk.wgrad(dh, b['xn'], G1, M, 4 * C, C, dt, label=pre + 'wg1')
             Bk.lane = ml
             Bk.gemm(dh, W[pre + self.NAMES['fc1'] + 'weight.T'], g, M, C, 4 * C, dt, label=pre + 'dg1')
-        du = self.tmp('du' + par, (M, C))
-        Bk.layernorm_bwd(g, b['xn'], None, b['rstd'], None, None, du, None, None, M, C, True, dt, label=pre + 'lnb')
+        if not ln_in:
+            Bk.layernorm_bwd(g, b['xn'], None, b['rstd'], None, None, du, None, None, M, C, True, dt, label=pre + 'lnb')
         dw49 = self.gbuf((49, C))
         Bk.lane = wl
         Bk.dwconv7_bwd_weight(du, b['x'], dw49, self.grad(pre + self.NAMES['dw'] + 'bias'), B, res, res, C, dt, label=pre + 'dww')
diff --git a/imagenet-models_amd/ops.py b/imagenet-models_amd/ops.py
--- a/imagenet-models_amd/ops.py
+++ b/imagenet-models_amd/ops.py
@@ -402,17 +402,21 @@
     def pad_copy(self, src, dst, rows, cols, lds, ldd, dtype, accumulate=False, label=None):
         self._add('ga_pad_copy', (_ptr(src), _ptr(dst), rows, cols, lds, ldd, int(accumulate), dtype), label, keep=(src, dst))
 
-    def mlp_fwd(self, X, W1, b1, W2, b2, Y, M, Cdim, dtype, ldw1=None, ldw2=None, R=None, rowscale=None, rows_per_scale=1, label=None):
+    def mlp_fwd(self, X, W1, b1, W2, b2, Y, M, Cdim, dtype, ldw1=None, ldw2=None, R=None, rowscale=None, rows_per_scale=1, label=None,
+                XN=None, RSTD=None, eps=0.0):
         d = L.MlpDesc()
         H = 4 * Cdim
         d.X, d.ldx, d.W1, d.ldw1, d.b1 = _ptr(X), Cdim, _ptr(W1), (Cdim if ldw1 is None else ldw1), _ptr(b1)
         d.W2, d.ldw2, d.b2 = _ptr(W2), (H if ldw2 is None else ldw2), _ptr(b2)
         d.R, d.ldr, d.rowscale, d.rows_per_scale = _ptr(R), Cdim, _ptr(rowscale), rows_per_scale
         d.Y, d.ldy, d.M, d.C, d.H, d.dtype = _ptr(Y), Cdim, M, Cdim, H, dtype
-        self._add('ga_mlp_fwd', (C.byref(d),), label, keep=(d, X, W1, b1, W2, b2, R, rowscale, Y))
+        if XN is not None or RSTD is not None:
+            assert RSTD is None or RSTD.dtype == torch.float32
+            d.eps, d.XN, d.ldxn, d.RSTD = eps, _ptr(XN), Cdim, _ptr(RSTD)
+        self._add('ga_mlp_fwd', (C.byref(d),), label, keep=(d, X, W1, b1, W2, b2, R, rowscale, Y, XN, RSTD))
 
     def mlp_bwd(self, X, DY, W1, b1, W2T, W1T, A, DH, DX, M, Cdim, dtype, ldw1=None, ldw2t=None, ldw1t=None, label=None,
-                dW1=None, db1=None, partials=None, max_blocks=0):
+                dW1=None, db1=None, partials=None, max_blocks=0, RSTD=None, DU=None):
         d = L.MlpBwdDesc()
         H = 4 * Cdim
         d.X, d.ldx, d.DY, d.lddy = _ptr(X), Cdim, _ptr(DY), Cdim
@@ -425,7 +429,10 @@
             assert dW1.stride(-1) == 1 and partials.dtype == torch.float32 and partials.is_contiguous()
             d.dW1, d.ldw, d.db1 = _ptr(dW1), dW1.stride(0), _ptr(db1)
             d.partials, d.partials_bytes, d.max_blocks = _ptr(partials), partials.numel() * 4, max_blocks
-        self._add('ga_mlp_bwd', (C.byref(d),), label, keep=(d, X, DY, W1, b1, W2T, W1T, A, DH, DX, dW1, db1, partials))
+        if DU is not None or RSTD is not None:
+            assert RSTD is None or RSTD.dtype == torch.float32
+            d.RSTD, d.DU, d.lddu = _ptr(RSTD), _ptr(DU), Cdim
+        self._add('ga_mlp_bwd', (C.byref(d),), label, keep=(d, X, DY, W1, b1, W2T, W1T, A, DH, DX, dW1, db1, partials, RSTD, DU))
 
     def wgrad(self, Y, X, dW, M, N, K, dtype, ldy=None, ldx=None, ldw=None, batch=1, strideY=0, strideX=0, strideW=0,
               x_kind=A_PLAIN, x_dims=(0, 0, 0), x_act=ACT_NONE, dbias=None, strideDbias=0, alpha=1.0, split_m=None,
@@ -901,6 +908,10 @@
     return bool(L.load().ga_mlp_supported(Cdim, H, dtype))
 
 
+def mlp_ln_supported(Cdim, H, dtype):
+    return bool(L.load().ga_mlp_ln_supported(Cdim, H, dtype))
+
+
 def mlp_bwd_wgrad_supported(Cdim, H, dtype):
     return bool(L.load().ga_mlp_bwd_wgrad_supported(Cdim, H, dtype))
 
diff --git a/include/gaext.h b/include/gaext.h
--- a/include/gaext.h
+++ b/include/gaext.h
@@ -335,6 +335,9 @@
     const float* rowscale; int rows_per_scale;
     void* Y; int64_t ldy;
     int64_t M; int C, H, dtype;
+    float eps;
+    void* XN; int64_t ldxn;
+    float* RSTD;
 } ga_mlp_desc;
 typedef struct {
     const void* X; int64_t ldx;
@@ -350,8 +353,11 @@
     float* db1;
     float* partials; size_t partials_bytes;
     int max_blocks;
+    const float* RSTD;
+    void* DU; int64_t lddu;
 } ga_mlp_bwd_desc;
 int ga_mlp_supported(int C, int H, int dtype);
+int ga_mlp_ln_supported(int C, int H, int dtype);
 int ga_mlp_fwd(const ga_mlp_desc* d, ga_stream_t stream);
 int ga_mlp_bwd(const ga_mlp_bwd_desc* d, ga_stream_t stream);
 int ga_mlp_bwd_wgrad_supported(int C, int H, int dtype);
```

After: 11000 images/sec. No clear change (-0.7%).
